# tooHotSpot/FGN

Measured on AMD Instinct MI355X. Metric: query-imgs/sec (3-way 3-shot, 800x1333 FGN simple_test), higher is better.
Workload: dtype f32; 1 GPU; cfg3: COCO2VOC 3-way 3-shot, query 3x800x1333, supports 9x3x256^2, ResNet-50-C4, R<=300 proposals, D<=100 detections, 1 episode(s) per GPU per step; h2d_in_step=True, gt_mask_rle_in_step=True, world_size_seen=1, phase_lock=rpn, caller_streams=2, support_cache=False, hip_graph=True, winograd_3x3=F(4x4,3x3)

## Files before the change

fgn_amd/csrc/common.h:

```cpp
#pragma once
#include <hip/hip_runtime.h>
#include <stdint.h>

#define FGN_OK 0
#define FGN_ERR_SHAPE (-1)
#define FGN_ERR_ARG (-2)

#define FGN_LAUNCH_CHECK()                         \
    do {                                           \
        hipError_t e__ = hipGetLastError();        \
        if (e__ != hipSuccess) return (int)e__;    \
    } while (0)

static inline int cdiv(int a, int b) { return (a + b - 1) / b; }

#include <hip/hip_ext.h>
extern thread_local hipEvent_t fgn_prof_start;
extern thread_local hipEvent_t fgn_prof_stop;
#define FGN_LAUNCH_TIMED(kernel, grid, block, lds, stream, ...)                                            \
    do {                                                                                                   \
        if (fgn_prof_start) {                                                                              \
            hipExtLaunchKernelGGL(kernel, grid, block, lds, stream, fgn_prof_start, fgn_prof_stop, 0, __VA_ARGS__); \
            fgn_prof_start = nullptr;                                                                      \
            fgn_prof_stop = nullptr;                                                                       \
        } else {                                                                                           \
            hipLaunchKernelGGL(kernel, grid, block, lds, stream, __VA_ARGS__);                             \
        }                                                                                                  \
    } while (0)

constexpr int FGN_STAMP_WORDS = 72;
extern thread_local unsigned long long* fgn_stamp_base;
extern thread_local int fgn_stamp_next, fgn_stamp_cap;
static inline unsigned long long* fgn_next_stamp_record() {
    if (!fgn_stamp_base || fgn_stamp_next >= fgn_stamp_cap) return nullptr;
    return fgn_stamp_base + FGN_STAMP_WORDS * (size_t)fgn_stamp_next++;
}

static inline hipError_t fgn_allow_full_lds(const void* fn, unsigned long long* done_mask) {
    int dev = 0;
    hipError_t e = hipGetDevice(&dev);
    if (e != hipSuccess) return e;
    if (dev < 64 && ((*done_mask >> dev) & 1ull)) return hipSuccess;
    e = hipFuncSetAttribute(fn, hipFuncAttributeMaxDynamicSharedMemorySize, 160 * 1024);
    if (e == hipSuccess && dev < 64) *done_mask |= 1ull << dev;
    return e;
}

typedef float f32x16 __attribute__((ext_vector_type(16)));
typedef float f32x4 __attribute__((ext_vector_type(4)));

__device__ __forceinline__ float wave_reduce_sum(float v) {
#pragma unroll
    for (int off = 32; off > 0; off >>= 1) v += __shfl_xor(v, off, 64);
    return v;
}
```

fgn_amd/csrc/conv_igemm.hip:

```cpp
#include "common.h"
#include <cstdlib>

struct ConvParams {
    const float* x = nullptr;
    const float* w = nullptr;
    float* y = nullptr;
    const float* scale = nullptr;
    const float* shift = nullptr;
    const float* residual = nullptr;
    const float* in_scale = nullptr;
    const int32_t* n_img_dev = nullptr;
    int n_img = 0, H = 1, W = 1, Cin = 0, Ho = 1, Wo = 1, Cout = 0, KH = 1, KW = 1, stride = 1, pad = 0;
    int a_img_div = 1;
    int relu = 0;
    int K = 0;
    int n_tiles_n = 0;
    int band_nt = 0, band_mt = 0;
    float* ws = nullptr;
    int splits = 1, kt_per_split = 0;
#ifdef FGN_EXPERIMENTS
    int32_t* tickets = nullptr;
    int32_t* sched = nullptr;
    int sk_U = 0, sk_dp = 0;
#endif
    unsigned x_bytes = 0, w_bytes = 0;
    int grp_rows = 0, grp_valid = 0, grp_items = 0, grp_rows_per_item = 0, grp_w_stride = 0;
    const int32_t* grp_count_dev = nullptr;
    unsigned long long* stamp = nullptr;
    const float* x2 = nullptr;
    unsigned x2_bytes = 0;
    int kt1 = 0, cin2 = 0;
    const int32_t* x2_rows = nullptr;
    const void* w3 = nullptr;
    unsigned w3_bytes = 0;
    int npad3 = 0;
    const float* w_inv = nullptr;
};

#ifndef CONV_DMA_STAGES
#define CONV_DMA_STAGES 2
#endif
constexpr int BK = 32;
constexpr int LDS_STRIDE = 36;

#ifdef CONV_CLOCK_STAMPS
__device__ unsigned long long g_clock_stamps[16384 * 6];
#define CLOCK_STAMP_BEGIN()                                                \
    const unsigned long long cs_t0 = __builtin_amdgcn_s_memtime();         \
    const unsigned long long cs_r0 = __builtin_amdgcn_s_memrealtime();     \
    __builtin_amdgcn_s_waitcnt(0xC07F)
#define CLOCK_STAMP_END(slot)                                              \
    do {                                                                   \
        const unsigned long long cs_t1 = __builtin_amdgcn_s_memtime();     \
        const unsigned long long cs_r1 = __builtin_amdgcn_s_memrealtime(); \
        __builtin_amdgcn_s_waitcnt(0xC07F);                                \
        unsigned cs_xcc, cs_hw;                                            \
        asm volatile("s_getreg_b32 %0, hwreg(HW_REG_XCC_ID)" : "=s"(cs_xcc)); \
        asm volatile("s_getreg_b32 %0, hwreg(HW_REG_HW_ID)" : "=s"(cs_hw));   \
        if (threadIdx.x == 0 && (slot) < 16384) {                          \
            g_clock_stamps[(slot) * 6 + 0] = cs_t0;                        \
            g_clock_stamps[(slot) * 6 + 1] = cs_t1;                        \
            g_clock_stamps[(slot) * 6 + 2] = cs_r0;                        \
            g_clock_stamps[(slot) * 6 + 3] = cs_r1;                        \
            g_clock_stamps[(slot) * 6 + 4] = cs_xcc;                       \
            g_clock_stamps[(slot) * 6 + 5] = cs_hw;                        \
        }                                                                  \
    } while (0)
#else
#define CLOCK_STAMP_BEGIN() do { } while (0)
#define CLOCK_STAMP_END(slot) do { } while (0)
#endif

template <int A_LD>
struct AStage {
    int off[A_LD];
    unsigned long long taps[A_LD];
    int soff[A_LD];
};

template <int N>
struct Pack {
    typedef float type __attribute__((ext_vector_type(N)));
};
#define PACK_SET4(pk, i, v)      \
    do {                         \
        (pk)[4 * (i) + 0] = (v).x; \
        (pk)[4 * (i) + 1] = (v).y; \
        (pk)[4 * (i) + 2] = (v).z; \
        (pk)[4 * (i) + 3] = (v).w; \
    } while (0)
#define PACK_GET4(pk, i) make_float4((pk)[4 * (i)], (pk)[4 * (i) + 1], (pk)[4 * (i) + 2], (pk)[4 * (i) + 3])

template <int A_LD, int B_LD, bool IN_SCALE>
__device__ __forceinline__ unsigned load_tile(const ConvParams& p, const AStage<A_LD>& st, const float* b_base,
                                              int kt, int cin_tiles, int col4,
                                              typename Pack<4 * A_LD>::type& a_reg,
                                              typename Pack<4 * A_LD>::type& s_reg,
                                              typename Pack<4 * B_LD>::type& b_reg) {
    unsigned ok_mask = 0;
    const int tap = kt / cin_tiles;
    const int c0 = (kt - tap * cin_tiles) * BK;
    const int ky = tap / p.KW, kx = tap - ky * p.KW;
    const int tap_off = (ky * p.W + kx) * p.Cin + c0;
#pragma unroll
    for (int i = 0; i < A_LD; ++i) {
        const bool ok = (st.taps[i] >> tap) & 1ull;
        const int off = ok ? st.off[i] + tap_off : 0;
        const float4 v = *reinterpret_cast<const float4*>(p.x + off);
        PACK_SET4(a_reg, i, v);
        if (IN_SCALE) {
            const float4 sv = *reinterpret_cast<const float4*>(p.in_scale + st.soff[i] + c0);
            PACK_SET4(s_reg, i, sv);
        }
        ok_mask |= ok ? (1u << i) : 0u;
    }
#pragma unroll
    for (int i = 0; i < B_LD; ++i) {
        const float4 v = *reinterpret_cast<const float4*>(b_base + (size_t)(32 * i) * p.K + kt * BK);
        PACK_SET4(b_reg, i, v);
    }
// ... 251 lines not shown
    constexpr unsigned OOB = 0x7ffffff0u;

    extern __shared__ __attribute__((aligned(16))) float smem[];

    const int t = threadIdx.x;
    const int lane = t & 63;
    const int wv = t >> 6;
    const int wm = wv / WAVES_N, wn = wv % WAVES_N;

    const int nwg = nwg_in;
    int bid = bx;
    {
        const int q = nwg >> 3, r = nwg & 7, xcd = bid & 7, idx = bid >> 3;
        bid = (xcd < r ? xcd * (q + 1) : r * (q + 1) + (xcd - r) * q) + idx;
    }
    int tile_m = bid / p.n_tiles_n;
    int tile_n = bid - tile_m * p.n_tiles_n;
    if (p.band_nt > 0) {
        const int per_grp = p.band_mt * p.n_tiles_n;
        const int grp = bid / per_grp;
        int r = bid - grp * per_grp;
        const int per_band = p.band_mt * p.band_nt;
        const int band = r / per_band;
        r -= band * per_band;
        const int mi = r / p.band_nt;
        tile_m = grp * p.band_mt + mi;
        tile_n = band * p.band_nt + (r - mi * p.band_nt);
    }
    const int m0 = tile_m * BM;
    const int n0 = tile_n * BN;

    const int HoWo = p.Ho * p.Wo;
    int n_img = p.n_img;
    if (p.n_img_dev) n_img = min(n_img, *p.n_img_dev);
    const int M = n_img * HoWo;
    if (m0 >= M) return;

    const int col4 = t & 7;
    const int row0 = t >> 3;
    const int src_c4 = col4 ^ ((row0 >> 1) & 7);
    int a_off[A_LD];
    unsigned long long a_taps[A_LD];
#pragma unroll
    for (int i = 0; i < A_LD; ++i) {
        const int m = m0 + row0 + 32 * i;
        a_off[i] = 0; a_taps[i] = 0ull;
        if (PW) {
            a_off[i] = (m * p.Cin + src_c4 * 4) * 4;
            a_taps[i] = m < M ? 1ull : 0ull;
        } else if (STEM) {
            if (m < M) {
                const int img = m / HoWo;
                const int rem = m - img * HoWo;
                const int oy = rem / p.Wo;
                const int ox = rem - oy * p.Wo;
                const int iy0 = oy * p.stride - p.pad, ix = ox * p.stride - p.pad + src_c4;
                a_off[i] = (((img / p.a_img_div) * p.H + iy0) * p.W + ix) * 16;
                unsigned long long tm = 0ull;
                if (src_c4 < p.KW && (unsigned)ix < (unsigned)p.W)
                    for (int ky = 0; ky < p.KH; ++ky)
                        if ((unsigned)(iy0 + ky) < (unsigned)p.H) tm |= 1ull << ky;
                a_taps[i] = tm;
            }
        } else if (m < M) {
            const int img = m / HoWo;
            const int rem = m - img * HoWo;
            const int oy = rem / p.Wo;
            const int ox = rem - oy * p.Wo;
            const int iy0 = oy * p.stride - p.pad, ix0 = ox * p.stride - p.pad;
            a_off[i] = ((((img / p.a_img_div) * p.H + iy0) * p.W + ix0) * p.Cin + src_c4 * 4) * 4;
            unsigned long long tm = 0ull;
            int tp = 0;
            for (int ky = 0; ky < p.KH; ++ky) {
                const bool y_ok = (unsigned)(iy0 + ky) < (unsigned)p.H;
                for (int kx = 0; kx < p.KW; ++kx, ++tp)
                    if (y_ok && (unsigned)(ix0 + kx) < (unsigned)p.W) tm |= 1ull << tp;
            }
            a_taps[i] = tm;
        }
    }
    int b_off0 = ((n0 + row0) * p.K + src_c4 * 4) * 4;
    if (PW && p.grp_rows) {
        const int grp = m0 / p.grp_rows;
        int valid = p.grp_valid;
        if (p.grp_count_dev) valid = min(valid, min(p.grp_items, *p.grp_count_dev) * p.grp_rows_per_item);
        if (m0 - grp * p.grp_rows >= valid) return;
        b_off0 += grp * p.grp_w_stride * 4;
    }

    const i32x4 x_rs = make_rsrc(p.x, p.x_bytes);
    const i32x4 w_rs = make_rsrc(p.w, p.w_bytes);

    const int KT_all = p.K / BK;
    const int kt0 = by * p.kt_per_split;
    const int KT = min(KT_all, kt0 + p.kt_per_split);
    const int cin_tiles = p.Cin / BK;

    const unsigned lds_base = __builtin_amdgcn_readfirstlane((unsigned)reinterpret_cast<size_t>(smem));
    const unsigned wave_row_bytes = __builtin_amdgcn_readfirstlane(wv) * 8 * 128;

    int nx_tap = 0, nx_c0t = 0, nx_kx = 0, nx_off = 0;
    if (!PW && !STEM) {
        nx_tap = kt0 / cin_tiles;
        nx_c0t = kt0 - nx_tap * cin_tiles;
        const int ky = nx_tap / p.KW;
        nx_kx = nx_tap - ky * p.KW;
        nx_off = ((ky * p.W + nx_kx) * p.Cin + nx_c0t * BK) * 4;
    }
    auto issue_tile = [&](int kt, int stage) {
        int tap = 0, tap_off = kt * BK * 4;
        if (STEM) {
            tap = kt;
            tap_off = kt * p.W * 16;
        } else if (!PW && NSTAGE == 2) {
            tap = nx_tap;
            tap_off = nx_off;
            nx_off += BK * 4;
            if (++nx_c0t == cin_tiles) {
                nx_c0t = 0;
                ++nx_tap;
                if (++nx_kx == p.KW) {
                    nx_kx = 0;
                    nx_off += (p.W - p.KW) * p.Cin * 4;
                }
            }
        } else if (!PW) {
            tap = kt / cin_tiles;
            const int c0 = (kt - tap * cin_tiles) * BK;
            const int ky = tap / p.KW, kx = tap - ky * p.KW;
            tap_off = ((ky * p.W + kx) * p.Cin + c0) * 4;
        }
        const unsigned sa = lds_base + stage * (STAGE * 4) + wave_row_bytes;
#pragma unroll
        for (int i = 0; i < A_LD; ++i) {
            const bool ok = (a_taps[i] >> tap) & 1ull;
            if (PW) {
                lds_dma16_s(x_rs, sa + i * 32 * 128, ok ? (unsigned)a_off[i] : OOB, (unsigned)tap_off);
                continue;
            }
            const unsigned voff = ok ? (unsigned)(a_off[i] + tap_off) : OOB;
            lds_dma16(x_rs, sa + i * 32 * 128, voff);
        }
        const unsigned sb = sa + BM * 128;
        const unsigned bko = (unsigned)(kt * BK * 4);
#pragma unroll
        for (int i = 0; i < B_LD; ++i)
            lds_dma16_s(w_rs, sb + i * 32 * 128, (unsigned)(b_off0 + i * 32 * p.K * 4), bko);
    };

    f32x16 acc[TM][TN];
#pragma unroll
    for (int i = 0; i < TM; ++i)
#pragma unroll
        for (int j = 0; j < TN; ++j)
#pragma unroll
            for (int r = 0; r < 16; ++r) acc[i][j][r] = 0.f;

    const int frag_row = lane & 31;
    const int half = lane >> 5;
    const int rswz = (frag_row >> 1) & 7;
    const float* const rd_a = smem + (wm * WM + frag_row) * BK;
    const float* const rd_b = smem + BM * BK + (wn * WN + frag_row) * BK;

#pragma unroll
    for (int s = 0; s < NSTAGE - 1; ++s) issue_tile(min(kt0 + s, KT - 1), s);
    if (NSTAGE == 2) asm volatile("s_waitcnt vmcnt(0)" ::: "memory");
    else asm volatile("s_waitcnt vmcnt(%0)" ::"n"(LOADS) : "memory");
    __builtin_amdgcn_s_barrier();
// ... 87 lines not shown
                        v.x = v.x * sc.x + sh.x; v.y = v.y * sc.y + sh.y; v.z = v.z * sc.z + sh.z; v.w = v.w * sc.w + sh.w;
                        v.x += res[k].x; v.y += res[k].y; v.z += res[k].z; v.w += res[k].w;
                        if (p.relu) {
                            v.x = fmaxf(v.x, 0.f); v.y = fmaxf(v.y, 0.f); v.z = fmaxf(v.z, 0.f); v.w = fmaxf(v.w, 0.f);
                        }
                    }
                    *reinterpret_cast<float4*>(dst + (size_t)m * p.Cout + n) = v;
                }
            }
        }
        return;
    }
    if (p.splits > 1) {
        float* slab = p.ws + (size_t)by * ((size_t)p.n_img * HoWo) * p.Cout;
#pragma unroll
        for (int j = 0; j < TN; ++j) {
            const int n = n0 + wn * WN + j * 32 + frag_row;
#pragma unroll
            for (int i = 0; i < TM; ++i) {
                const int mb = m0 + wm * WM + i * 32 + 4 * half;
#pragma unroll
                for (int r = 0; r < 16; ++r) {
                    const int m = mb + (r & 3) + 8 * (r >> 2);
                    if (n < p.Cout && m < M) slab[(size_t)m * p.Cout + n] = acc[i][j][r];
                }
            }
        }
        return;
    }
#pragma unroll
    for (int j = 0; j < TN; ++j) {
        const int n = n0 + wn * WN + j * 32 + frag_row;
        const bool n_ok = n < p.Cout;
        const float sc = (n_ok && p.scale) ? p.scale[n] : 1.f;
        const float sh = (n_ok && p.shift) ? p.shift[n] : 0.f;
#pragma unroll
        for (int i = 0; i < TM; ++i) {
            const int mb = m0 + wm * WM + i * 32 + 4 * half;
#pragma unroll
            for (int r = 0; r < 16; ++r) {
                const int m = mb + (r & 3) + 8 * (r >> 2);
                if (n_ok && m < M) {
                    const size_t o = (size_t)m * p.Cout + n;
                    float v = acc[i][j][r] * sc + sh;
                    if (p.residual) v += p.residual[o];
                    if (p.relu) v = fmaxf(v, 0.f);
                    p.y[o] = v;
                }
            }
        }
    }
}

template <int BM, int BN, int WM, int WN, int NSTAGE, int MIN_WAVES, int MODE>
__global__ __launch_bounds__(256, MIN_WAVES) void conv_igemm_dma_kernel(const ConvParams p) {
    CLOCK_STAMP_BEGIN();
    conv_igemm_dma_body<BM, BN, WM, WN, NSTAGE, MODE>(p, blockIdx.x, gridDim.x, blockIdx.y);
#ifdef CONV_CLOCK_STAMPS
    asm volatile("s_waitcnt vmcnt(0)" ::: "memory");
#endif
    CLOCK_STAMP_END(blockIdx.x);
}

template <int BM, int BN, int WM, int WN, int NSTAGE, int MIN_WAVES, int MODE>
__global__ __launch_bounds__(256, MIN_WAVES) void conv_igemm_dma_pair_kernel(const ConvParams p0, const ConvParams p1,
                                                                             const int n0) {
    if ((int)blockIdx.x < n0)
        conv_igemm_dma_body<BM, BN, WM, WN, NSTAGE, MODE>(p0, blockIdx.x, n0, 0);
    else
        conv_igemm_dma_body<BM, BN, WM, WN, NSTAGE, MODE>(p1, (int)blockIdx.x - n0, (int)gridDim.x - n0, 0);
}


__global__ __launch_bounds__(256, 5) void conv_pw_persist_kernel(const ConvParams p, const int total_tiles) {
    constexpr int BM = 64, BN = 64, WN = 32, WM = 32;
    constexpr int A_LD = 2, B_LD = 2;
    constexpr int STAGE = (BM + BN) * BK;
    constexpr int PITCH = BN;
    extern __shared__ __attribute__((aligned(16))) float smem[];

    const int t = threadIdx.x, lane = t & 63, wv = t >> 6;
    const int wm = wv >> 1, wn = wv & 1;
    const int M = (p.n_img_dev ? min(p.n_img, *p.n_img_dev) : p.n_img) * p.Ho * p.Wo;
    int grp_valid = p.grp_valid;
    if (p.grp_rows && p.grp_count_dev) grp_valid = min(grp_valid, min(p.grp_items, *p.grp_count_dev) * p.grp_rows_per_item);

    const int col4 = t & 7, row0 = t >> 3;
    const int src_c4 = col4 ^ ((row0 >> 1) & 7);
    const i32x4 x_rs = make_rsrc(p.x, p.x_bytes);
    const i32x4 w_rs = make_rsrc(p.w, p.w_bytes);
    const bool dual = p.x2 != nullptr;
    const i32x4 x2_rs = make_rsrc(dual ? p.x2 : p.x, dual ? p.x2_bytes : p.x_bytes);
    const int KT = p.K / BK;
    const unsigned lds_base = __builtin_amdgcn_readfirstlane((unsigned)reinterpret_cast<size_t>(smem));
    const unsigned wave_row_bytes = __builtin_amdgcn_readfirstlane(wv) * 8 * 128;
    constexpr unsigned OOB = 0x7ffffff0u;

    const int nq = total_tiles >> 3, nr = total_tiles & 7;
    auto coords = [&](int tile, int& m0, int& n0) -> bool {
        const int xcd = tile & 7, idx = tile >> 3;
        const int bid = (xcd < nr ? xcd * (nq + 1) : nr * (nq + 1) + (xcd - nr) * nq) + idx;
        int tile_m = bid / p.n_tiles_n;
        int tile_n = bid - tile_m * p.n_tiles_n;
        if (p.band_nt > 0) {
            const int per_grp = p.band_mt * p.n_tiles_n;
            const int grp = bid / per_grp;
            int r = bid - grp * per_grp;
            const int per_band = p.band_mt * p.band_nt;
            const int band = r / per_band;
            r -= band * per_band;
            const int mi = r / p.band_nt;
            tile_m = grp * p.band_mt + mi;
            tile_n = band * p.band_nt + (r - mi * p.band_nt);
        }
        m0 = tile_m * BM;
        n0 = tile_n * BN;
        if (m0 >= M) return false;
        if (p.grp_rows && m0 - (m0 / p.grp_rows) * p.grp_rows >= grp_valid) return false;
        return true;
    };
    auto next_active = [&](int tile, int& m0, int& n0) -> int {
        for (; tile < total_tiles; tile += gridDim.x)
            if (coords(tile, m0, n0)) return tile;
        return -1;
    };

    unsigned a_voff[A_LD], a2_voff[A_LD], b_voff[B_LD];
    auto set_offsets = [&](int m0, int n0) {
#pragma unroll
        for (int i = 0; i < A_LD; ++i) {
            const int m = m0 + row0 + 32 * i;
            a_voff[i] = m < M ? (unsigned)((m * p.Cin + src_c4 * 4) * 4) : OOB;
            a2_voff[i] = OOB;
            if (dual && m < M) a2_voff[i] = (unsigned)(((p.x2_rows ? p.x2_rows[m] : m) * p.cin2 + src_c4 * 4) * 4);
        }
        int b0 = ((n0 + row0) * p.K + src_c4 * 4) * 4;
        if (p.grp_rows) b0 += (m0 / p.grp_rows) * p.grp_w_stride * 4;
#pragma unroll
        for (int i = 0; i < B_LD; ++i) b_voff[i] = (unsigned)(b0 + i * 32 * p.K * 4);
    };
    auto issue_tile = [&](int kt, int stage) {
        const unsigned sa = lds_base + stage * (STAGE * 4) + wave_row_bytes;
        const unsigned ko = (unsigned)(kt * BK * 4);
        if (dual && kt >= p.kt1) {
            const unsigned ko2 = (unsigned)((kt - p.kt1) * BK * 4);
#pragma unroll
            for (int i = 0; i < A_LD; ++i) lds_dma16_s(x2_rs, sa + i * 32 * 128, a2_voff[i], ko2);
        } else {
#pragma unroll
            for (int i = 0; i < A_LD; ++i) lds_dma16_s(x_rs, sa + i * 32 * 128, a_voff[i], ko);
        }
        const unsigned sb = sa + BM * 128;
#pragma unroll
        for (int i = 0; i < B_LD; ++i) lds_dma16_s(w_rs, sb + i * 32 * 128, b_voff[i], ko);
    };

    const int r16 = lane & 15, g16 = lane >> 4;
    const float* const rd_a = smem + (wm * WM + r16) * BK;
    const float* const rd_b = smem + BM * BK + (wn * WN + r16) * BK;
    float* const cbase = smem + STAGE;

    if (p.stamp && t == 0 && blockIdx.x == 0) atomicExch(p.stamp, __builtin_amdgcn_s_memrealtime());
    auto leave = [&]() {
        if (!p.stamp || t != 0) return;
        const unsigned shard = blockIdx.x & 7u;
        const unsigned long long in_shard = (gridDim.x - shard + 7u) / 8u;
        unsigned long long* const sc = p.stamp + 8 * (1 + shard);
        if (atomicAdd(sc, 1ull) != in_shard - 1) return;
        atomicExch(sc, 0ull);
        const unsigned long long shards = gridDim.x < 8u ? gridDim.x : 8u;
        if (atomicAdd(p.stamp + 2, 1ull) != shards - 1) return;
        const unsigned long long d = __builtin_amdgcn_s_memrealtime() - atomicExch(p.stamp, 0ull);
        atomicExch(p.stamp + 2, 0ull);
        atomicAdd(p.stamp + 1, d);
        atomicAdd(p.stamp + 3, 1ull);
        atomicMin(p.stamp + 4, d);
        atomicMax(p.stamp + 5, d);
    };
    int m0, n0;
    int tile = next_active(blockIdx.x, m0, n0);
    if (tile < 0) { leave(); return; }
    CLOCK_STAMP_BEGIN();
    set_offsets(m0, n0);
    issue_tile(0, 0);

    while (true) {
        f32x4 acc4[2][2];
#pragma unroll
        for (int i = 0; i < 2; ++i)
#pragma unroll
            for (int j = 0; j < 2; ++j) acc4[i][j] = f32x4{0.f, 0.f, 0.f, 0.f};
        asm volatile("s_waitcnt vmcnt(0) lgkmcnt(0)" ::: "memory");
        __builtin_amdgcn_s_barrier();
        int cur = 0;
        for (int kt = 0; kt < KT; ++kt) {
            if (kt + 1 < KT) issue_tile(kt + 1, cur ^ 1);
            asm volatile("" ::: "memory");
            const float* As = rd_a + cur * STAGE;
            const float* Bs = rd_b + cur * STAGE;
#pragma unroll
            for (int kk = 0; kk < 2; ++kk) {
// ... 644 lines not shown
                                         const float* w_packed, float* y, const float* shift, int rows, int Cin1, int Cin2,
                                         int Cout, int cout_pad, int relu, hipStream_t stream) {
    ConvParams p;
    const int rc = describe_dual(p, MATH_F32, x, x2, x2_rows, x2_total_rows, w_packed, y, shift, rows, Cin1, Cin2, Cout, cout_pad, relu);
    if (rc != FGN_DESCRIBED) return rc;
    p.n_tiles_n = cdiv(Cout, 64);
    const int m_tiles = cdiv(rows, 64);
    set_band(p, 64, m_tiles, 64ll * p.K * 4);
    return launch_persist(p, m_tiles * p.n_tiles_n, stream);
}

extern "C" int fgn_conv1x1_dual_x3_nhwc_f32(const float* x, const float* x2, const int32_t* x2_rows, int x2_total_rows,
                                            const void* w_x3, float* y, const float* shift, int rows, int Cin1, int Cin2,
                                            int Cout, int cout_pad, int relu, hipStream_t stream) {
    ConvParams p;
    const int rc = describe_dual(p, MATH_X3, x, x2, x2_rows, x2_total_rows, w_x3, y, shift, rows, Cin1, Cin2, Cout, cout_pad, relu);
    if (rc != FGN_DESCRIBED) return rc;
    return launch_x3(p, rows, 0, 6, stream);
}

extern "C" int fgn_conv1x1_dual_h2_nhwc_f32(const float* x, const float* x2, const int32_t* x2_rows, int x2_total_rows,
                                            const void* w_h2, float* y, const float* shift, int rows, int Cin1, int Cin2,
                                            int Cout, int cout_pad, int relu, hipStream_t stream) {
    ConvParams p;
    const int rc = describe_dual(p, MATH_H2, x, x2, x2_rows, x2_total_rows, w_h2, y, shift, rows, Cin1, Cin2, Cout, cout_pad, relu);
    if (rc != FGN_DESCRIBED) return rc;
    return launch_h2(p, rows, 1, 0, stream);
}
extern "C" int fgn_conv1x1_dual_h2_bm_nhwc_f32(const float* x, const float* x2, const int32_t* x2_rows, int x2_total_rows,
                                               const void* w_h2, float* y, const float* shift, int rows, int Cin1, int Cin2,
                                               int Cout, int cout_pad, int relu, int bm, hipStream_t stream) {
    ConvParams p;
    const int rc = describe_dual(p, MATH_H2, x, x2, x2_rows, x2_total_rows, w_h2, y, shift, rows, Cin1, Cin2, Cout, cout_pad, relu);
    if (rc != FGN_DESCRIBED) return rc;
    return launch_h2(p, rows, 1, bm, stream);
}

static int describe_gemm(ConvParams& p, const GemmMath& m, const float* x, const void* w, float* y, const float* shift,
                         const float* residual, int rows, int K, int Cout, int npad, int relu, int grp_rows, int grp_valid,
                         int n_groups) {
    if (!x || !w || !y) return FGN_ERR_ARG;
    if (rows <= 0) return FGN_OK;
    if (K % BK || K <= 0 || (Cout & 3) || npad % m.bn || npad < Cout || n_groups < 1) return FGN_ERR_SHAPE;
    if (n_groups > 1 && (grp_rows <= 0 || (long long)n_groups * grp_rows != rows || grp_valid > grp_rows)) return FGN_ERR_SHAPE;
    const long long xb = (long long)rows * K * 4, wb = gemm_weight_bytes(m, K, npad, n_groups);
    if (xb >= 0x7fffff00ll || wb >= 0x7fffff00ll || (long long)rows * Cout >= (1ll << 31)) return FGN_ERR_SHAPE;
    p.x = x; p.y = y; p.shift = shift; p.residual = residual;
    p.n_img = rows; p.Cin = K; p.Cout = Cout; p.relu = relu; p.K = K; p.kt_per_split = K / BK; p.x_bytes = (unsigned)xb;
    p.grp_rows = n_groups > 1 ? grp_rows : 0; p.grp_valid = grp_valid;
    gemm_set_weights(p, m, w, wb, npad);
    return FGN_DESCRIBED;
}

extern "C" int fgn_gemm_x3_f32(const float* x, const void* w3, float* y, const float* shift, const float* residual,
                               int rows, int K, int Cout, int npad, int relu, int grp_rows, int grp_valid, int n_groups,
                               int bm, int nterms, hipStream_t stream) {
    ConvParams p;
    const int rc = describe_gemm(p, MATH_X3, x, w3, y, shift, residual, rows, K, Cout, npad, relu, grp_rows, grp_valid, n_groups);
    if (rc != FGN_DESCRIBED) return rc;
#ifdef X3_PHASES
    if (!g_x3_ph && (hipMalloc(&g_x3_ph, 256) != hipSuccess || hipMemset(g_x3_ph, 0, 256) != hipSuccess)) return FGN_ERR_ARG;
    p.ws = reinterpret_cast<float*>(g_x3_ph);
#endif
    return launch_x3(p, rows, bm, nterms, stream);
}

extern "C" int fgn_gemm_h2_f32(const float* x, const void* w_h2, float* y, const float* shift, const float* residual,
                               int rows, int K, int Cout, int npad, int relu, int grp_rows, int grp_valid, int n_groups,
                               int bm, hipStream_t stream) {
    ConvParams p;
    const int rc = describe_gemm(p, MATH_H2, x, w_h2, y, shift, residual, rows, K, Cout, npad, relu, grp_rows, grp_valid, n_groups);
    if (rc != FGN_DESCRIBED) return rc;
#ifdef H2_PHASES
    if (!g_x3_ph && (hipMalloc(&g_x3_ph, 256) != hipSuccess || hipMemset(g_x3_ph, 0, 256) != hipSuccess)) return FGN_ERR_ARG;
    p.ws = reinterpret_cast<float*>(g_x3_ph);
#endif
    return launch_h2(p, rows, n_groups, bm, stream);
}

extern "C" int fgn_winograd_t_pad(int tiles_total) { return (tiles_total + 127) / 128 * 128; }

static int describe_winograd_gemm(ConvParams& p, const GemmMath& m, const float* V, const void* U, float* Mo,
                                  const int32_t* n_img_dev, int n_img, int tiles_per_img, int t_pad, int Cin, int Cout,
                                  int cout_pad, int n_groups) {
    if (!V || !U || !Mo) return FGN_ERR_ARG;
    if (n_img <= 0) return FGN_OK;
    if (Cin % BK != 0 || (m.deep && Cin < 2 * BK) || Cout % 4 != 0 || cout_pad % m.bn != 0 || cout_pad < Cout || t_pad % 64 != 0 ||
        (n_groups != 16 && n_groups != 36) || (long long)n_img * tiles_per_img > t_pad)
        return FGN_ERR_SHAPE;
    const long long rows = (long long)n_groups * t_pad;
    const long long xb = rows * Cin * 4, wb = gemm_weight_bytes(m, Cin, cout_pad, n_groups);
    if (xb >= 0x7fffff00ll || wb >= 0x7fffff00ll || rows * Cout >= (1ll << 31)) return FGN_ERR_SHAPE;
    p.x = V; p.y = Mo;
    p.n_img = (int)rows; p.Cin = Cin; p.Cout = Cout; p.K = Cin; p.kt_per_split = Cin / BK; p.x_bytes = (unsigned)xb;
    p.grp_rows = t_pad; p.grp_valid = n_img * tiles_per_img; p.grp_items = n_img;
    p.grp_rows_per_item = tiles_per_img; p.grp_count_dev = n_img_dev;
    gemm_set_weights(p, m, U, wb, cout_pad);
    if (!m.image_bytes) p.grp_w_stride = cout_pad * Cin;
    return FGN_DESCRIBED;
}

extern "C" int fgn_winograd_gemm_f32(const float* V, const float* U, float* Mo, const int32_t* n_img_dev, int n_img,
                                     int tiles_per_img, int t_pad, int Cin, int Cout, int cout_pad, int n_groups,
                                     hipStream_t stream) {
    ConvParams p;
    const int rc = describe_winograd_gemm(p, MATH_F32, V, U, Mo, n_img_dev, n_img, tiles_per_img, t_pad, Cin, Cout, cout_pad, n_groups);
    if (rc != FGN_DESCRIBED) return rc;
#ifdef FGN_EXPERIMENTS
    {
        int rc2 = FGN_OK;
        if (fgn_exp_pointwise(p, p.n_img, 4, true, t_pad, stream, &rc2)) return rc2;
    }
#endif
    return launch_cfg<64, 64, 32, 32, 4>(p, p.n_img, pointwise_mode(4, p.n_img, Cout, 1), stream);
}

extern "C" int fgn_winograd_gemm_x3_f32(const float* V, const void* U_x3, float* Mo, const int32_t* n_img_dev, int n_img,
                                        int tiles_per_img, int t_pad, int Cin, int Cout, int cout_pad, int n_groups,
                                        hipStream_t stream) {
    ConvParams p;
    const int rc = describe_winograd_gemm(p, MATH_X3, V, U_x3, Mo, n_img_dev, n_img, tiles_per_img, t_pad, Cin, Cout, cout_pad, n_groups);
    if (rc != FGN_DESCRIBED) return rc;
    return launch_x3(p, p.n_img, 0, 6, stream);
}

extern "C" int fgn_winograd_gemm_h2_f32(const float* V, const void* U_h2, float* Mo, const int32_t* n_img_dev, int n_img,
                                        int tiles_per_img, int t_pad, int Cin, int Cout, int cout_pad, int n_groups,
                                        hipStream_t stream) {
    ConvParams p;
    const int rc = describe_winograd_gemm(p, MATH_H2, V, U_h2, Mo, n_img_dev, n_img, tiles_per_img, t_pad, Cin, Cout, cout_pad, n_groups);
    if (rc != FGN_DESCRIBED) return rc;
    return launch_h2(p, p.n_img, n_groups, 0, stream);
}
```

fgn_amd/csrc/conv_pw_h2.h:

```cpp
#pragma once

typedef _Float16 f16x8_t __attribute__((ext_vector_type(8)));

struct H2Frag { f16x8_t hi, lo; };

__device__ __forceinline__ void h2_split4(const float x0, const float x1, const float x2, const float x3, const float s,
                                          unsigned& h01, unsigned& h23, unsigned& l01, unsigned& l23) {
    asm("v_fma_mixlo_f16 %0, %4, %8, 0\n\t"
        "v_fma_mixlo_f16 %1, %6, %8, 0\n\t"
        "v_fma_mixhi_f16 %0, %5, %8, 0\n\t"
        "v_fma_mixhi_f16 %1, %7, %8, 0\n\t"
        "v_fma_mixlo_f16 %2, %4, %8, -%0 op_sel:[0,0,0] op_sel_hi:[0,0,1]\n\t"
        "v_fma_mixlo_f16 %3, %6, %8, -%1 op_sel:[0,0,0] op_sel_hi:[0,0,1]\n\t"
        "v_fma_mixhi_f16 %2, %5, %8, -%0 op_sel:[0,0,1] op_sel_hi:[0,0,1]\n\t"
        "v_fma_mixhi_f16 %3, %7, %8, -%1 op_sel:[0,0,1] op_sel_hi:[0,0,1]\n\t"
        "s_nop 1"
        : "=&v"(h01), "=&v"(h23), "=&v"(l01), "=&v"(l23)
        : "v"(x0), "v"(x1), "v"(x2), "v"(x3), "s"(s));
}

__device__ __forceinline__ void h2_split4_step(const int step, const float x0, const float x1, const float x2, const float x3,
                                               const float s, unsigned& h01, unsigned& h23, unsigned& l01, unsigned& l23) {
    if (step == 0)
        asm("v_fma_mixlo_f16 %0, %2, %4, 0\n\t"
// ... 13 lines not shown
            : "+v"(l01), "+v"(l23) : "v"(x1), "v"(x3), "s"(s), "v"(h01), "v"(h23));
}

__device__ __forceinline__ H2Frag h2_split(const float4& a, const float4& b, const float s) {
    unsigned h[4], l[4];
    h2_split4(a.x, a.y, a.z, a.w, s, h[0], h[1], l[0], l[1]);
    h2_split4(b.x, b.y, b.z, b.w, s, h[2], h[3], l[2], l[3]);
    H2Frag f;
    f.hi = __builtin_bit_cast(f16x8_t, make_uint4(h[0], h[1], h[2], h[3]));
    f.lo = __builtin_bit_cast(f16x8_t, make_uint4(l[0], l[1], l[2], l[3]));
    return f;
}

__device__ __forceinline__ float h2_absmax16(const float4& a, const float4& b, const float4& c, const float4& d) {
    float m;
    asm("v_max3_f32 %0, |%1|, |%2|, 0\n\t"
        "v_max3_f32 %0, |%3|, |%4|, %0\n\t"
        "v_max3_f32 %0, |%5|, |%6|, %0\n\t"
        "v_max3_f32 %0, |%7|, |%8|, %0\n\t"
        "v_max3_f32 %0, |%9|, |%10|, %0\n\t"
        "v_max3_f32 %0, |%11|, |%12|, %0\n\t"
        "v_max3_f32 %0, |%13|, |%14|, %0\n\t"
        "v_max3_f32 %0, |%15|, |%16|, %0"
        : "=&v"(m)
        : "v"(a.x), "v"(a.y), "v"(a.z), "v"(a.w), "v"(b.x), "v"(b.y), "v"(b.z), "v"(b.w),
          "v"(c.x), "v"(c.y), "v"(c.z), "v"(c.w), "v"(d.x), "v"(d.y), "v"(d.z), "v"(d.w));
    return m;
}

constexpr int H2_BN = 128;

struct H2Im2col {
    float* y1;
    unsigned x_off0, x_off1;
    int M0, M1;
    int H1, W1, Ho1, Wo1;
    int cin_shift;
};

#ifdef H2_PHASES
#define H2_T(i) do { const unsigned long long now_ = __builtin_amdgcn_s_memtime(); ph_[i] += now_ - last_; last_ = now_; } while (0)
#else
#define H2_T(i) do { } while (0)
#endif
struct H2Yes { static constexpr bool value = true; };
struct H2No { static constexpr bool value = false; };
constexpr int H2_ONE = 0, H2_TWO = 1, H2_EITHER = 2;
template <int WMW, int WNW, int RB, int NST, bool IM2COL, int KG, int DUAL>
__device__ __forceinline__ void conv_pw_h2_body(const ConvParams p, const H2Im2col q2, const int total_tiles) {
    static_assert(!(DUAL != H2_ONE && IM2COL), "the implicit-GEMM loader reads one operand");
    constexpr int BM = 32 * RB * WMW, BN = 64 * WNW, NW = WMW * WNW, NTHR_G = 64 * NW, NTHR = NTHR_G * KG;
    static_assert(KG == 1 || KG == 2, "one or two K-groups");
    constexpr int A_LD = BM / 8 / NW;
    constexpr int A_STAGE = BM * 128;
    constexpr int B_STAGE = 2 * BN * 64;
    constexpr int STAGE = A_STAGE + B_STAGE;
    constexpr int BQ = BN / 16;
    constexpr int B_LD = 2 * BQ / NW;
    static_assert(A_LD * 8 * NW == BM && B_LD * NW == 2 * BQ, "tile / wave split");
    constexpr int PER = A_LD + B_LD;
    constexpr int ROWS_PER_PASS = NTHR_G / 8;
    constexpr bool OLD_CURSOR = KG == 2 && !IM2COL;
#ifdef H2_EPILOGUE_PASSES
    constexpr bool WPE = false;
#else
    constexpr bool WPE = KG == 1;
#endif
#ifdef H2_PHASES
    constexpr bool PEEL = true;
#else
    constexpr bool PEEL = WPE;
#endif
    constexpr int C_LD = 68;
    static_assert(!WPE || NW * 16 * C_LD * 4 <= STAGE, "a 16-row block per wave fits the free stage");
    static_assert(NST == 2, "a ring of two stages: one K-tile in flight ahead of the one being multiplied");
    extern __shared__ __attribute__((aligned(16))) unsigned char smem_h2[];

    const int t = threadIdx.x, lane = t & 63;
    const int kg = KG == 1 ? 0 : __builtin_amdgcn_readfirstlane((t >> 6) / NW);
    const int wv = KG == 1 ? t >> 6 : (t >> 6) % NW;
    const int tg = KG == 1 ? t : t % NTHR_G;
    const int wm = wv / WNW, wn = wv % WNW;
    const int M = IM2COL ? q2.M0 + q2.M1 : (p.n_img_dev ? min(p.n_img, *p.n_img_dev) : p.n_img) * p.Ho * p.Wo;
    int grp_valid = p.grp_valid;
    if (p.grp_rows && p.grp_count_dev) grp_valid = min(grp_valid, min(p.grp_items, *p.grp_count_dev) * p.grp_rows_per_item);

    float a_s = 1.f, a_inv = 1.f;

    const int col4 = tg & 7, row0 = tg >> 3;
    const int src_c4 = col4 ^ ((row0 >> 1) & 7);
    const i32x4 x_rs = make_rsrc(p.x, p.x_bytes);
    const i32x4 w_rs = make_rsrc(p.w3, p.w3_bytes);
    [[maybe_unused]] const bool dual = DUAL == H2_EITHER ? p.x2 != nullptr : DUAL == H2_TWO;
    [[maybe_unused]] const i32x4 x2_rs = DUAL != H2_ONE ? make_rsrc(dual ? p.x2 : p.x, dual ? p.x2_bytes : p.x_bytes) : x_rs;
    const int KT = p.K / BK / KG;
    const unsigned kt_bytes = (unsigned)(2 * p.npad3 * 64);
    const unsigned lds_base = __builtin_amdgcn_readfirstlane((unsigned)reinterpret_cast<size_t>(smem_h2) + kg * (NST * STAGE));
    const unsigned wave_row_bytes = __builtin_amdgcn_readfirstlane(wv) * 8 * 128;
    constexpr unsigned OOB = 0x7ffffff0u;

    const int nq = total_tiles >> 3, nr = total_tiles & 7;
    auto coords = [&](int tile, int& m0, int& n0) -> bool {
        const int xcd = tile & 7, idx = tile >> 3;
        const int bid = (xcd < nr ? xcd * (nq + 1) : nr * (nq + 1) + (xcd - nr) * nq) + idx;
        int tile_m = bid / p.n_tiles_n;
        int tile_n = bid - tile_m * p.n_tiles_n;
        if (p.band_nt > 0) {
            const int per_grp = p.band_mt * p.n_tiles_n;
            const int grp = bid / per_grp;
            int r = bid - grp * per_grp;
            const int per_band = p.band_mt * p.band_nt;
            const int band = r / per_band;
            r -= band * per_band;
            const int mi = r / p.band_nt;
            tile_m = grp * p.band_mt + mi;
            tile_n = band * p.band_nt + (r - mi * p.band_nt);
        }
        m0 = tile_m * BM;
        n0 = tile_n * BN;
        if (m0 >= M) return false;
        if (p.grp_rows && m0 - (m0 / p.grp_rows) * p.grp_rows >= grp_valid) return false;
        return true;
    };
    auto next_active = [&](int tile, int& m0, int& n0) -> int {
        for (; tile < total_tiles; tile += gridDim.x)
            if (coords(tile, m0, n0)) return tile;
        return -1;
    };

    constexpr int A2_LD = (IM2COL || DUAL != H2_ONE) ? A_LD : 1;
    struct Offs { unsigned a[A_LD], a2[A2_LD], b[B_LD]; };
    unsigned b_lds[B_LD];
#pragma unroll
    for (int i = 0; i < B_LD; ++i) {
        const int q = wv + NW * i;
        b_lds[i] = __builtin_amdgcn_readfirstlane((unsigned)(A_STAGE + (q / BQ) * (BN * 64) + (q % BQ) * 1024));
    }
    auto offsets = [&](int m0, int n0) -> Offs {
        Offs o;
        o.a2[0] = 0u;
        const int g_end = p.grp_rows ? (m0 / p.grp_rows) * p.grp_rows + grp_valid : M;
#pragma unroll
        for (int i = 0; i < A_LD; ++i) {
            const int m = m0 + row0 + ROWS_PER_PASS * i;
            if constexpr (IM2COL) {
                o.a[i] = 0u; o.a2[i] = 0u;
                if (m < M) {
                    const bool t1 = m >= q2.M0;
                    const int mm = t1 ? m - q2.M0 : m;
                    const int H = t1 ? q2.H1 : p.H, W = t1 ? q2.W1 : p.W, Wo = t1 ? q2.Wo1 : p.Wo;
                    const int HoWo = (t1 ? q2.Ho1 : p.Ho) * Wo;
                    const int img = mm / HoWo;
                    const int rem = mm - img * HoWo;
                    const int oy = rem / Wo;
                    const int ox = rem - oy * Wo;
                    const int iy0 = oy * p.stride - p.pad, ix0 = ox * p.stride - p.pad;
                    o.a[i] = (t1 ? q2.x_off1 : q2.x_off0) + (unsigned)((((img * H + iy0) * W + ix0) * p.Cin + src_c4 * 4) * 4);
                    unsigned tm = t1 ? 0x80000000u : 0u;
                    int tp = 0;
                    for (int ky = 0; ky < p.KH; ++ky) {
                        const bool y_ok = (unsigned)(iy0 + ky) < (unsigned)H;
                        for (int kx = 0; kx < p.KW; ++kx, ++tp)
                            if (y_ok && (unsigned)(ix0 + kx) < (unsigned)W) tm |= 1u << tp;
                    }
                    o.a2[i] = tm;
                }
                continue;
            }
            const bool in = m < M && m < g_end;
            o.a[i] = in ? (unsigned)((m * p.Cin + src_c4 * 4) * 4) : OOB;
            if constexpr (DUAL != H2_ONE) {
                o.a2[i] = OOB;
                if (dual && in) o.a2[i] = (unsigned)(((p.x2_rows ? p.x2_rows[m] : m) * p.cin2 + src_c4 * 4) * 4);
            }
        }
        unsigned g0 = 0;
        if (p.grp_rows) g0 = (unsigned)(m0 / p.grp_rows) * (unsigned)(KT * KG) * kt_bytes;
#pragma unroll
        for (int i = 0; i < B_LD; ++i) {
            const int q = wv + NW * i;
            const int plane = q / BQ, row = (q % BQ) * 16 + (lane >> 2);
            o.b[i] = g0 + (unsigned)(((plane * p.npad3 + n0 + row) * 4 + (lane & 3)) * 16);
        }
        return o;
    };
    const unsigned ko_step = (unsigned)(KG * BK * 4), kb_step = (unsigned)KG * kt_bytes;
    [[maybe_unused]] const unsigned ko1 = (DUAL != H2_ONE && dual) ? (unsigned)(p.kt1 * BK * 4) : 0xffffffffu;
    unsigned c_ko = 0u, c_kb = 0u;
    int c_tap = 0, c_cs = 0, c_kx = 0;
    unsigned c_off0 = 0u, c_off1 = 0u;
    const int im_ct = 1 << q2.cin_shift;
    const unsigned im_skip0 = (unsigned)((p.W - p.KW) * p.Cin * 4), im_skip1 = (unsigned)((q2.W1 - p.KW) * p.Cin * 4);
    auto seek = [&](int step) {
        const int kt = step * KG + kg;
        c_ko = (unsigned)(kt * BK * 4);
        c_kb = (unsigned)kt * kt_bytes;
        if constexpr (IM2COL) {
            c_tap = kt >> q2.cin_shift;
            c_cs = kt - (c_tap << q2.cin_shift);
            const int ky = p.KW == 3 ? (c_tap * 43) >> 7 : c_tap;
            c_kx = c_tap - ky * p.KW;
            c_off0 = (unsigned)(((ky * p.W + c_kx) * p.Cin + c_cs * BK) * 4);
            c_off1 = (unsigned)(((ky * q2.W1 + c_kx) * p.Cin + c_cs * BK) * 4);
        }
    };
    auto advance = [&]() {
        c_ko += ko_step;
        c_kb += kb_step;
        if constexpr (IM2COL) {
#pragma unroll
            for (int g = 0; g < KG; ++g) {
                const bool tw = ++c_cs == im_ct;
                c_cs = tw ? 0 : c_cs;
                c_tap += tw;
                c_kx += tw;
                const bool rw = c_kx == p.KW;
                c_kx = rw ? 0 : c_kx;
                c_off0 += 128u + (rw ? im_skip0 : 0u);
                c_off1 += 128u + (rw ? im_skip1 : 0u);
            }
        }
    };
    auto piece = [&](const Offs& o, const unsigned wr, const int idx) {
        const unsigned st = lds_base + wr;
// ... 419 lines not shown
```

fgn_amd/csrc/conv_pw_x3.h:

```cpp
#pragma once

typedef __bf16 bf16x8_t __attribute__((ext_vector_type(8)));

struct X3Frag { bf16x8_t p1, p2, p3; };

__device__ __forceinline__ X3Frag x3_split(const float4& lo, const float4& hi) {
    const float x[8] = {lo.x, lo.y, lo.z, lo.w, hi.x, hi.y, hi.z, hi.w};
    unsigned q1[4], q2[4], q3[4];
#pragma unroll
    for (int i = 0; i < 4; ++i) {
        const unsigned u0 = __float_as_uint(x[2 * i]), u1 = __float_as_uint(x[2 * i + 1]);
        q1[i] = __builtin_amdgcn_perm(u1, u0, 0x07060302u);
        const float r0 = x[2 * i] - __uint_as_float(u0 & 0xffff0000u);
        const float r1 = x[2 * i + 1] - __uint_as_float(u1 & 0xffff0000u);
        const unsigned v0 = __float_as_uint(r0), v1 = __float_as_uint(r1);
        q2[i] = __builtin_amdgcn_perm(v1, v0, 0x07060302u);
        const float s0 = r0 - __uint_as_float(v0 & 0xffff0000u);
        const float s1 = r1 - __uint_as_float(v1 & 0xffff0000u);
        q3[i] = __builtin_amdgcn_perm(__float_as_uint(s1), __float_as_uint(s0), 0x07060302u);
    }
    X3Frag f;
    f.p1 = __builtin_bit_cast(bf16x8_t, make_uint4(q1[0], q1[1], q1[2], q1[3]));
    f.p2 = __builtin_bit_cast(bf16x8_t, make_uint4(q2[0], q2[1], q2[2], q2[3]));
    f.p3 = __builtin_bit_cast(bf16x8_t, make_uint4(q3[0], q3[1], q3[2], q3[3]));
    return f;
}

constexpr int X3_BN = 128;
constexpr int X3_B_STAGE = 3 * X3_BN * 64;

#ifdef X3_PHASES
#define X3_T(i) do { const unsigned long long now_ = __builtin_amdgcn_s_memtime(); ph_[i] += now_ - last_; last_ = now_; } while (0)
#else
#define X3_T(i) do { } while (0)
#endif

template <int N> __device__ __forceinline__ void x3_wait_vm() { asm volatile("s_waitcnt vmcnt(%0)" ::"n"(N) : "memory"); }

template <int WMW, int RB, int NT, int NST, bool SH16>
__global__ __launch_bounds__(128 * WMW, 2) void conv_pw_x3_kernel(const ConvParams p, const int total_tiles) {
    constexpr int BM = 32 * RB * WMW, BN = X3_BN, NTHR = 128 * WMW, NW = 2 * WMW;
    constexpr int A_LD = BM / 8 / NW;
    constexpr int A_STAGE = BM * 128;
    constexpr int STAGE = A_STAGE + X3_B_STAGE;
    constexpr int B_LD = 24 / NW;
    constexpr int PER = A_LD + B_LD;
    constexpr int D = NST - 1;
    constexpr int ROWS_PER_PASS = NTHR / 8;
    static_assert(NST == 2 || NST == 3, "ring of 2 or 3 stages");
    extern __shared__ __attribute__((aligned(16))) unsigned char smem_x3[];

    const int t = threadIdx.x, lane = t & 63, wv = t >> 6;
    const int wm = wv >> 1, wn = wv & 1;
    const int M = (p.n_img_dev ? min(p.n_img, *p.n_img_dev) : p.n_img) * p.Ho * p.Wo;
    int grp_valid = p.grp_valid;
    if (p.grp_rows && p.grp_count_dev) grp_valid = min(grp_valid, min(p.grp_items, *p.grp_count_dev) * p.grp_rows_per_item);

    const int col4 = t & 7, row0 = t >> 3;
    const int src_c4 = col4 ^ ((row0 >> 1) & 7);
    const i32x4 x_rs = make_rsrc(p.x, p.x_bytes);
    const i32x4 w_rs = make_rsrc(p.w3, p.w3_bytes);
    const bool dual = p.x2 != nullptr;
    const i32x4 x2_rs = make_rsrc(dual ? p.x2 : p.x, dual ? p.x2_bytes : p.x_bytes);
    const int KT = p.K / BK;
    const unsigned kt_bytes = (unsigned)(3 * p.npad3 * 64);
    const unsigned lds_base = __builtin_amdgcn_readfirstlane((unsigned)reinterpret_cast<size_t>(smem_x3));
    const unsigned wave_row_bytes = __builtin_amdgcn_readfirstlane(wv) * 8 * 128;
    constexpr unsigned OOB = 0x7ffffff0u;

    const int nq = total_tiles >> 3, nr = total_tiles & 7;
    auto coords = [&](int tile, int& m0, int& n0) -> bool {
        const int xcd = tile & 7, idx = tile >> 3;
        const int bid = (xcd < nr ? xcd * (nq + 1) : nr * (nq + 1) + (xcd - nr) * nq) + idx;
        int tile_m = bid / p.n_tiles_n;
        int tile_n = bid - tile_m * p.n_tiles_n;
        if (p.band_nt > 0) {
            const int per_grp = p.band_mt * p.n_tiles_n;
            const int grp = bid / per_grp;
            int r = bid - grp * per_grp;
            const int per_band = p.band_mt * p.band_nt;
            const int band = r / per_band;
            r -= band * per_band;
            const int mi = r / p.band_nt;
            tile_m = grp * p.band_mt + mi;
            tile_n = band * p.band_nt + (r - mi * p.band_nt);
        }
        m0 = tile_m * BM;
        n0 = tile_n * BN;
        if (m0 >= M) return false;
        if (p.grp_rows && m0 - (m0 / p.grp_rows) * p.grp_rows >= grp_valid) return false;
        return true;
    };
    auto next_active = [&](int tile, int& m0, int& n0) -> int {
        for (; tile < total_tiles; tile += gridDim.x)
            if (coords(tile, m0, n0)) return tile;
        return -1;
    };

    struct Offs { unsigned a[A_LD], a2[A_LD], b[B_LD]; };
    unsigned b_lds[B_LD];
#pragma unroll
    for (int i = 0; i < B_LD; ++i) {
        const int q = wv + NW * i;
        b_lds[i] = __builtin_amdgcn_readfirstlane((unsigned)(A_STAGE + (q >> 3) * (BN * 64) + (q & 7) * 1024));
    }
    auto offsets = [&](int m0, int n0) -> Offs {
        Offs o;
#pragma unroll
        for (int i = 0; i < A_LD; ++i) {
            const int m = m0 + row0 + ROWS_PER_PASS * i;
            o.a[i] = m < M ? (unsigned)((m * p.Cin + src_c4 * 4) * 4) : OOB;
            o.a2[i] = OOB;
            if (dual && m < M) o.a2[i] = (unsigned)(((p.x2_rows ? p.x2_rows[m] : m) * p.cin2 + src_c4 * 4) * 4);
        }
        unsigned g0 = 0;
        if (p.grp_rows) g0 = (unsigned)(m0 / p.grp_rows) * (unsigned)KT * kt_bytes;
#pragma unroll
        for (int i = 0; i < B_LD; ++i) {
            const int q = wv + NW * i;
            const int plane = q >> 3, row = (q & 7) * 16 + (lane >> 2);
            o.b[i] = g0 + (unsigned)(((plane * p.npad3 + n0 + row) * 4 + (lane & 3)) * 16);
        }
        return o;
    };
    auto issue = [&](const Offs& o, int kt, int stage) {
        const unsigned st = lds_base + stage * STAGE;
        const unsigned sa = st + wave_row_bytes;
        const unsigned ko = (unsigned)(kt * BK * 4);
        if (dual && kt >= p.kt1) {
            const unsigned ko2 = (unsigned)((kt - p.kt1) * BK * 4);
#pragma unroll
            for (int i = 0; i < A_LD; ++i) lds_dma16_s(x2_rs, sa + i * ROWS_PER_PASS * 128, o.a2[i], ko2);
        } else {
#pragma unroll
            for (int i = 0; i < A_LD; ++i) lds_dma16_s(x_rs, sa + i * ROWS_PER_PASS * 128, o.a[i], ko);
        }
        const unsigned kb = (unsigned)kt * kt_bytes;
#pragma unroll
        for (int i = 0; i < B_LD; ++i) lds_dma16_s(w_rs, st + b_lds[i], o.b[i], kb);
    };

    const int r32 = lane & 31, h = lane >> 5;
    const int a_row = wm * 32 * RB + r32;
    const unsigned a_sw = (unsigned)((a_row >> 1) & 7);
    unsigned a_rd[2][2], b_rd[2][2];
#pragma unroll
    for (int s = 0; s < 2; ++s) {
        const unsigned ca = (unsigned)(4 * s + 2 * h);
        a_rd[s][0] = (unsigned)(a_row * 128) + ((ca ^ a_sw) << 4);
        a_rd[s][1] = (unsigned)(a_row * 128) + (((ca + 1) ^ a_sw) << 4);
#pragma unroll
        for (int j = 0; j < 2; ++j) {
            const int n = wn * 64 + 32 * j + r32;
            b_rd[s][j] = (unsigned)(A_STAGE + n * 64) + ((((unsigned)(2 * s + h)) ^ (unsigned)((n >> 2) & 3)) << 4);
        }
    }

    const int r16 = lane & 15, g4 = lane >> 4;
    const int a16_row = wm * 32 * RB + r16;
    const unsigned a16_sw = (unsigned)((a16_row >> 1) & 7);
    const unsigned a16_rd0 = (unsigned)(a16_row * 128) + ((((unsigned)g4) ^ a16_sw) << 4);
    const unsigned a16_rd1 = (unsigned)(a16_row * 128) + ((((unsigned)(g4 + 4)) ^ a16_sw) << 4);
    const int n16 = wn * 64 + r16;
    const unsigned tau16 = (0x1230u >> (4 * ((n16 >> 2) & 3))) & 3u;
    const unsigned b16_rd = (unsigned)(A_STAGE + n16 * 64) + ((((unsigned)g4) ^ tau16) << 4);

    if (p.stamp && t == 0 && blockIdx.x == 0) atomicExch(p.stamp, __builtin_amdgcn_s_memrealtime());
    auto leave = [&]() {
        if (!p.stamp || t != 0) return;
        const unsigned shard = blockIdx.x & 7u;
        const unsigned long long in_shard = (gridDim.x - shard + 7u) / 8u;
        unsigned long long* const sc = p.stamp + 8 * (1 + shard);
        if (atomicAdd(sc, 1ull) != in_shard - 1) return;
// ... 233 lines not shown
```

fgn_amd/csrc/winograd.hip:

```cpp
#include "common.h"
#include <cstdlib>

__device__ __forceinline__ float4 f4add(float4 a, float4 b) { return make_float4(a.x + b.x, a.y + b.y, a.z + b.z, a.w + b.w); }
__device__ __forceinline__ float4 f4sub(float4 a, float4 b) { return make_float4(a.x - b.x, a.y - b.y, a.z - b.z, a.w - b.w); }
__device__ __forceinline__ float4 f4mul(float4 a, float4 b) { return make_float4(a.x * b.x, a.y * b.y, a.z * b.z, a.w * b.w); }

__global__ __launch_bounds__(256) void wg_input_kernel(const float4* __restrict__ x, const float4* __restrict__ in_scale,
                                                       float4* __restrict__ V, const int32_t* __restrict__ n_img_dev,
                                                       int n_img, int a_img_div, int H, int W, int C4, int ty, int tx,
                                                       int t_pad, long long total) {
    if (n_img_dev) n_img = min(n_img, *n_img_dev);
    for (long long i = blockIdx.x * (long long)blockDim.x + threadIdx.x; i < total;
         i += (long long)gridDim.x * blockDim.x) {
        const int c = (int)(i % C4);
        const int t = (int)(i / C4);
        const int xx = t % tx;
        const int r = t / tx;
        const int yy = r % ty;
        const int img = r / ty;
        if (img >= n_img) break;
        const float4* src = x + (size_t)(img / a_img_div) * H * W * C4 + c;
        const int iy0 = 2 * yy - 1, ix0 = 2 * xx - 1;
        float4 d[4][4];
#pragma unroll
// ... 85 lines not shown
    if (n_img <= 0) return FGN_OK;
    const int ty = (H + 1) / 2, tx = (W + 1) / 2;
    if (C % 4 != 0 || a_img_div < 1 || H < 1 || W < 1 || (long long)n_img * ty * tx > t_pad) return FGN_ERR_SHAPE;
    const long long total = (long long)n_img * ty * tx * (C / 4);
    const int grid = (int)std::min<long long>((total + 255) / 256, 256 * 32);
    FGN_LAUNCH_TIMED(wg_input_kernel, dim3(grid), dim3(256), 0, stream, reinterpret_cast<const float4*>(x),
                       reinterpret_cast<const float4*>(in_scale), reinterpret_cast<float4*>(V), n_img_dev, n_img,
                       a_img_div, H, W, C / 4, ty, tx, t_pad, total);
    FGN_LAUNCH_CHECK();
    return FGN_OK;
}

extern "C" int fgn_winograd_output_f32(const float* Mo, float* y, const float* shift, const int32_t* n_img_dev,
                                       int n_img, int H, int W, int C, int t_pad, int relu, hipStream_t stream) {
    if (!Mo || !y) return FGN_ERR_ARG;
    if (n_img <= 0) return FGN_OK;
    const int ty = (H + 1) / 2, tx = (W + 1) / 2;
    if (C % 4 != 0 || (long long)n_img * ty * tx > t_pad) return FGN_ERR_SHAPE;
    const long long total = (long long)n_img * ty * tx * (C / 4);
    const int grid = (int)std::min<long long>((total + 255) / 256, 256 * 32);
    FGN_LAUNCH_TIMED(wg_output_kernel, dim3(grid), dim3(256), 0, stream, reinterpret_cast<const float4*>(Mo),
                       reinterpret_cast<float4*>(y), reinterpret_cast<const float4*>(shift), n_img_dev, n_img, H, W,
                       C / 4, ty, tx, t_pad, relu, total);
    FGN_LAUNCH_CHECK();
    return FGN_OK;
}

template <int V>
struct VF {
    typedef float type __attribute__((ext_vector_type(V)));
};
template <int V>
using vf = typename VF<V>::type;

template <int V>
__device__ __forceinline__ vf<V> vfma(float k, vf<V> a, vf<V> acc) {
    vf<V> r;
#pragma unroll
    for (int i = 0; i < V; ++i) r[i] = fmaf(k, a[i], acc[i]);
    return r;
}
template <int V>
__device__ __forceinline__ vf<V> vmul_rn(vf<V> a, vf<V> s) {
#pragma clang fp contract(off)
    return a * s;
}
template <int V>
__device__ __forceinline__ vf<V> vzero() {
    vf<V> r;
#pragma unroll
    for (int i = 0; i < V; ++i) r[i] = 0.f;
    return r;
}
template <int V>
__device__ __forceinline__ vf<V> vrelu(vf<V> a) {
#pragma unroll
    for (int i = 0; i < V; ++i) a[i] = fmaxf(a[i], 0.f);
    return a;
}
template <int V>
__device__ __forceinline__ void wg4_bt(const vf<V> (&d)[6], vf<V> (&r)[6]) {
    r[0] = (vfma<V>(1.5f, d[3] - d[1], vfma<V>(-2.f, d[2], d[0]))) + d[4];
    r[1] = vfma<V>(2.5f, d[3], vfma<V>(0.5f, d[2], d[4] - d[1]));
    r[2] = vfma<V>(0.5f, d[3], vfma<V>(-2.5f, d[2], d[1] + d[4]));
    r[3] = vfma<V>(2.f, d[3] - d[1], d[4] - d[2]);
    r[4] = vfma<V>(0.5f, d[1] - d[3], d[4] - d[2]);
    r[5] = (vfma<V>(1.5f, d[4] - d[2], vfma<V>(-2.f, d[3], d[1]))) + d[5];
}
template <int V>
__device__ __forceinline__ void wg4_at(const vf<V> (&m)[6], vf<V> (&r)[4]) {
    const vf<V> s12 = m[1] + m[2], d12 = m[1] - m[2];
    r[0] = (m[0] + s12) + (m[3] + m[4]);
    r[1] = vfma<V>(-2.f, m[4], vfma<V>(0.5f, m[3], d12));
    r[2] = vfma<V>(4.f, m[4], vfma<V>(0.25f, m[3], s12));
    r[3] = (vfma<V>(-8.f, m[4], vfma<V>(0.125f, m[3], d12))) + m[5];
}

struct WgSeg {
    const float* x;
    int n_img, H, W, ty, tx;
    int tiles0;
};

template <int V, bool EAGER>
__global__ __launch_bounds__(256) void wg4_input_kernel(const float* __restrict__ x_, const float* __restrict__ in_scale_,
                                                        float* __restrict__ V_, const int32_t* __restrict__ n_img_dev,
                                                        int n_img, int a_img_div, int H, int W, int CV, int ty, int tx,
                                                        int t_pad, long long total, const WgSeg seg) {
    typedef vf<V> T;
    const T* __restrict__ x = reinterpret_cast<const T*>(x_);
    const T* __restrict__ in_scale = reinterpret_cast<const T*>(in_scale_);
    T* __restrict__ Vo = reinterpret_cast<T*>(V_);
    if (n_img_dev) n_img = min(n_img, *n_img_dev);
    for (long long i = blockIdx.x * (long long)blockDim.x + threadIdx.x; i < total;
         i += (long long)gridDim.x * blockDim.x) {
        const int c = (int)(i % CV);
        const int t = (int)(i / CV);
        const bool second = seg.x && t >= seg.tiles0;
        if (second) {
            x = reinterpret_cast<const T*>(seg.x);
            H = seg.H; W = seg.W; ty = seg.ty; tx = seg.tx; n_img = seg.n_img; a_img_div = 1;
        }
        const int tl = second ? t - seg.tiles0 : t;
        const int xx = tl % tx;
        const int r = tl / tx;
        const int yy = r % ty;
        const int img = r / ty;
        if (img >= n_img) {
            if (seg.x) continue;
            break;
        }
        const T* src = x + (size_t)(img / a_img_div) * H * W * CV + c;
        const int iy0 = 4 * yy - 1, ix0 = 4 * xx - 1;
        T s;
        if (in_scale) s = in_scale[(size_t)img * CV + c];
        else {
#pragma unroll
            for (int k = 0; k < V; ++k) s[k] = 1.f;
        }
        T tt[6][6];
        if (EAGER) {
#pragma unroll
            for (int a = 0; a < 6; ++a) {
                const int iy = iy0 + a;
#pragma unroll
                for (int b = 0; b < 6; ++b) {
                    const int ix = ix0 + b;
                    tt[a][b] = ((unsigned)iy < (unsigned)H && (unsigned)ix < (unsigned)W)
                                   ? src[((size_t)iy * W + ix) * CV] : vzero<V>();
                }
            }
#pragma unroll
            for (int b = 0; b < 6; ++b) {
                T d[6], rr[6];
#pragma unroll
                for (int a = 0; a < 6; ++a) d[a] = vmul_rn<V>(tt[a][b], s);
                wg4_bt<V>(d, rr);
#pragma unroll
                for (int a = 0; a < 6; ++a) tt[a][b] = rr[a];
            }
        } else {
#pragma unroll
            for (int b = 0; b < 6; ++b) {
                const int ix = ix0 + b;
                T d[6], rr[6];
#pragma unroll
                for (int a = 0; a < 6; ++a) {
                    const int iy = iy0 + a;
                    d[a] = ((unsigned)iy < (unsigned)H && (unsigned)ix < (unsigned)W)
                               ? vmul_rn<V>(src[((size_t)iy * W + ix) * CV], s) : vzero<V>();
                }
                wg4_bt<V>(d, rr);
#pragma unroll
                for (int a = 0; a < 6; ++a) tt[a][b] = rr[a];
            }
        }
        T* dst = Vo + (size_t)t * CV + c;
        const size_t gs = (size_t)t_pad * CV;
#pragma unroll
        for (int a = 0; a < 6; ++a) {
            T rr[6];
            wg4_bt<V>(tt[a], rr);
#pragma unroll
            for (int b = 0; b < 6; ++b) dst[(a * 6 + b) * gs] = rr[b];
        }
    }
}

template <int V>
__global__ __launch_bounds__(256) void wg4_output_kernel(const float* __restrict__ Mo_, float* __restrict__ y_,
                                                         const float* __restrict__ shift_,
                                                         const int32_t* __restrict__ n_img_dev, int n_img, int H, int W,
                                                         int CV, int ty, int tx, int t_pad, int relu, long long total,
                                                         const WgSeg seg) {
    typedef vf<V> T;
    const T* __restrict__ Mo = reinterpret_cast<const T*>(Mo_);
    const T* __restrict__ shift = reinterpret_cast<const T*>(shift_);
    T* __restrict__ y = reinterpret_cast<T*>(y_);
    if (n_img_dev) n_img = min(n_img, *n_img_dev);
    for (long long i = blockIdx.x * (long long)blockDim.x + threadIdx.x; i < total;
         i += (long long)gridDim.x * blockDim.x) {
        const int c = (int)(i % CV);
        const int t = (int)(i / CV);
        const bool second = seg.x && t >= seg.tiles0;
        if (second) {
            y = reinterpret_cast<T*>(const_cast<float*>(seg.x));
            H = seg.H; W = seg.W; ty = seg.ty; tx = seg.tx; n_img = seg.n_img;
        }
        const int tl = second ? t - seg.tiles0 : t;
        const int xx = tl % tx;
        const int r = tl / tx;
        const int yy = r % ty;
        const int img = r / ty;
        if (img >= n_img) {
            if (seg.x) continue;
            break;
        }
        const T* src = Mo + (size_t)t * CV + c;
        const size_t gs = (size_t)t_pad * CV;
        T mm[6][6];
#pragma unroll
        for (int a = 0; a < 6; ++a)
#pragma unroll
            for (int b = 0; b < 6; ++b) mm[a][b] = src[(a * 6 + b) * gs];
        T st[4][6];
#pragma unroll
        for (int b = 0; b < 6; ++b) {
            T m[6], rr[4];
#pragma unroll
            for (int a = 0; a < 6; ++a) m[a] = mm[a][b];
            wg4_at<V>(m, rr);
#pragma unroll
            for (int k = 0; k < 4; ++k) st[k][b] = rr[k];
        }
        const T sh = shift ? shift[c] : vzero<V>();
#pragma unroll
        for (int a = 0; a < 4; ++a) {
            const int oy = 4 * yy + a;
            T rr[4];
            wg4_at<V>(st[a], rr);
            if (oy >= H) continue;
#pragma unroll
            for (int b = 0; b < 4; ++b) {
                const int ox = 4 * xx + b;
                if (ox >= W) continue;
                T v = rr[b] + sh;
                if (relu) v = vrelu<V>(v);
                y[(((size_t)img * H + oy) * W + ox) * CV + c] = v;
            }
        }
    }
}

struct WgDiv {
    uint32_t mul, shift;
};
static WgDiv wg_div(uint32_t d) {
    WgDiv r = {0u, 0u};
    if (d > 1) {
        const int L = 32 - __builtin_clz(d - 1);
        r.mul = (uint32_t)(((1ull << (31 + L)) + d - 1) / d);
        r.shift = (uint32_t)(L - 1);
    }
    return r;
}
__device__ __forceinline__ uint32_t wg_quot(uint32_t n, WgDiv d) { return d.mul ? __umulhi(n, d.mul) >> d.shift : n; }

struct WgMap {
    const float* p;
    int H, W;
    int n_img;
    uint32_t ty, tx;
    WgDiv dty, dtx;
    uint32_t elems;
};
struct WgNarrow {
    WgMap m[2];
    uint32_t blocks0;
    uint32_t tiles0;
    uint32_t CV;
    WgDiv dcv, ddiv;
    uint32_t gs;
};

template <typename T>
__device__ __forceinline__ T wg_ld(const void* base, uint32_t off) {
    return *reinterpret_cast<const T*>(static_cast<const char*>(base) + off);
}
template <typename T>
__device__ __forceinline__ void wg_st(void* base, uint32_t off, T v) {
    *reinterpret_cast<T*>(static_cast<char*>(base) + off) = v;
}

__device__ __forceinline__ int wg_count_early(const int32_t* n_img_dev) {
    if (!n_img_dev) return 0x7fffffff;
    const int32_t* p = n_img_dev;
    asm volatile("" : "+v"(p));
    return *p;
}

template <int V>
__global__ __launch_bounds__(256) void wg4_input_narrow_kernel(const WgNarrow P, const float* __restrict__ in_scale,
                                                               float* __restrict__ Vo, const int32_t* __restrict__ n_img_dev) {
    typedef vf<V> T;
    const int dev_count = wg_count_early(n_img_dev);
    const bool second = blockIdx.x >= P.blocks0;
    const float* __restrict__ x = second ? P.m[1].p : P.m[0].p;
    const int H = second ? P.m[1].H : P.m[0].H, W = second ? P.m[1].W : P.m[0].W;
    const uint32_t ty = second ? P.m[1].ty : P.m[0].ty, tx = second ? P.m[1].tx : P.m[0].tx;
    const WgDiv dty = second ? P.m[1].dty : P.m[0].dty, dtx = second ? P.m[1].dtx : P.m[0].dtx;
    const uint32_t elems = second ? P.m[1].elems : P.m[0].elems;
    const int n_cap = second ? P.m[1].n_img : P.m[0].n_img;
    const uint32_t i = (blockIdx.x - (second ? P.blocks0 : 0u)) * 256u + threadIdx.x;
    if (i >= elems) return;
    const uint32_t tl = wg_quot(i, P.dcv), c = i - tl * P.CV;
    const uint32_t r = wg_quot(tl, dtx), xx = tl - r * tx;
    const uint32_t img = wg_quot(r, dty), yy = r - img * ty;
    const uint32_t t = tl + (second ? P.tiles0 : 0u);
    const uint32_t px = (uint32_t)sizeof(T) * P.CV;
    const int iy0 = 4 * (int)yy - 1, ix0 = 4 * (int)xx - 1;
    uint32_t ro[6], co[6];
    bool rok[6], cok[6];
    const uint32_t row0 = wg_quot(img, P.ddiv) * (uint32_t)H;
#pragma unroll
    for (int a = 0; a < 6; ++a) {
        const int iy = iy0 + a, ix = ix0 + a;
        rok[a] = (unsigned)iy < (unsigned)H;
        cok[a] = (unsigned)ix < (unsigned)W;
        ro[a] = (row0 + (uint32_t)min(max(iy, 0), H - 1)) * (uint32_t)W * px;
        co[a] = (uint32_t)min(max(ix, 0), W - 1) * px + c * (uint32_t)sizeof(T);
    }
    T tt[6][6];
#pragma unroll
    for (int a = 0; a < 6; ++a)
#pragma unroll
        for (int b = 0; b < 6; ++b) tt[a][b] = wg_ld<T>(x, ro[a] + co[b]);
    T s;
    if (in_scale) s = wg_ld<T>(in_scale, (img * P.CV + c) * (uint32_t)sizeof(T));
    else {
#pragma unroll
        for (int k = 0; k < V; ++k) s[k] = 1.f;
    }
#pragma unroll
    for (int b = 0; b < 6; ++b) {
        T d[6], rr[6];
#pragma unroll
        for (int a = 0; a < 6; ++a) d[a] = vmul_rn<V>((rok[a] && cok[b]) ? tt[a][b] : vzero<V>(), s);
        wg4_bt<V>(d, rr);
#pragma unroll
        for (int a = 0; a < 6; ++a) tt[a][b] = rr[a];
    }
    if ((int)img >= min(n_cap, dev_count)) return;
    uint32_t o = (t * P.CV + c) * (uint32_t)sizeof(T);
#pragma unroll
    for (int a = 0; a < 6; ++a) {
        T rr[6];
        wg4_bt<V>(tt[a], rr);
#pragma unroll
        for (int b = 0; b < 6; ++b) {
            wg_st<T>(Vo, o, rr[b]);
            o += P.gs;
        }
    }
}

template <int V>
__global__ __launch_bounds__(256) void wg4_output_narrow_kernel(const WgNarrow P, const float* __restrict__ Mo,
                                                                const float* __restrict__ shift,
                                                                const int32_t* __restrict__ n_img_dev, int relu) {
    typedef vf<V> T;
    const int dev_count = wg_count_early(n_img_dev);
    const bool second = blockIdx.x >= P.blocks0;
    float* __restrict__ y = const_cast<float*>(second ? P.m[1].p : P.m[0].p);
    const int H = second ? P.m[1].H : P.m[0].H, W = second ? P.m[1].W : P.m[0].W;
    const uint32_t ty = second ? P.m[1].ty : P.m[0].ty, tx = second ? P.m[1].tx : P.m[0].tx;
    const WgDiv dty = second ? P.m[1].dty : P.m[0].dty, dtx = second ? P.m[1].dtx : P.m[0].dtx;
    const uint32_t elems = second ? P.m[1].elems : P.m[0].elems;
    const int n_cap = second ? P.m[1].n_img : P.m[0].n_img;
    const uint32_t i = (blockIdx.x - (second ? P.blocks0 : 0u)) * 256u + threadIdx.x;
    if (i >= elems) return;
    const uint32_t tl = wg_quot(i, P.dcv), c = i - tl * P.CV;
    const uint32_t t = tl + (second ? P.tiles0 : 0u);
    T mm[6][6];
    {
        uint32_t o = (t * P.CV + c) * (uint32_t)sizeof(T);
#pragma unroll
        for (int a = 0; a < 6; ++a)
#pragma unroll
            for (int b = 0; b < 6; ++b) {
                mm[a][b] = wg_ld<T>(Mo, o);
                o += P.gs;
            }
    }
    const T sh = shift ? wg_ld<T>(shift, c * (uint32_t)sizeof(T)) : vzero<V>();
    const uint32_t r = wg_quot(tl, dtx), xx = tl - r * tx;
    const uint32_t img = wg_quot(r, dty), yy = r - img * ty;
    T st[4][6];
#pragma unroll
    for (int b = 0; b < 6; ++b) {
        T m[6], rr[4];
#pragma unroll
        for (int a = 0; a < 6; ++a) m[a] = mm[a][b];
        wg4_at<V>(m, rr);
#pragma unroll
        for (int k = 0; k < 4; ++k) st[k][b] = rr[k];
    }
    if ((int)img >= min(n_cap, dev_count)) return;
    const uint32_t px = (uint32_t)sizeof(T) * P.CV;
    const uint32_t oy0 = 4u * yy, ox0 = 4u * xx;
    uint32_t orow = ((img * (uint32_t)H + oy0) * (uint32_t)W + ox0) * px + c * (uint32_t)sizeof(T);
#pragma unroll
    for (int a = 0; a < 4; ++a) {
        T rr[4];
        wg4_at<V>(st[a], rr);
        if ((int)(oy0 + a) < H) {
#pragma unroll
            for (int b = 0; b < 4; ++b) {
                if ((int)(ox0 + b) >= W) continue;
                T v = rr[b] + sh;
                if (relu) v = vrelu<V>(v);
                wg_st<T>(y, orow + b * px, v);
            }
        }
        orow += (uint32_t)W * px;
    }
}

static int wg4_vec(long long elems) { return elems >= (4ll << 20) ? 4 : 2; }
static bool wg4_eager(long long) { return true; }
extern "C" int fgn_winograd4_variant(int tiles_total, int C, int is_output) {
    const int v = wg4_vec((long long)tiles_total * C);
    return v * 10 + ((!is_output && wg4_eager((long long)tiles_total * (C / v))) ? 1 : 0);
}

static bool wg4_narrow_fits(long long imgs0, int H0, int W0, long long imgs1, int H1, int W1, long long n_scale, int C,
                            int t_pad) {
    const long long lim = 0x7fffffffll, cb = 4ll * C;
    return imgs0 * H0 * W0 * cb <= lim && imgs1 * H1 * W1 * cb <= lim && n_scale * cb <= lim && 36ll * t_pad * cb <= lim;
}
static void wg4_map(WgMap& m, const float* p, int n_img, int H, int W, int cv) {
    m.p = p; m.H = H; m.W = W; m.n_img = n_img;
    m.ty = (uint32_t)(H + 3) / 4; m.tx = (uint32_t)(W + 3) / 4;
    m.dty = wg_div(m.ty); m.dtx = wg_div(m.tx);
    m.elems = p ? (uint32_t)n_img * m.ty * m.tx * (uint32_t)cv : 0u;
}
static WgNarrow wg4_narrow(const float* p0, int n_img0, int a_img_div, int H0, int W0, const float* p1, int n_img1, int H1,
                           int W1, int C, int vec, int t_pad, int* grid) {
    WgNarrow P;
    const int cv = C / vec;
    wg4_map(P.m[0], p0, n_img0, H0, W0, cv);
    wg4_map(P.m[1], p1, n_img1, H1, W1, cv);
    P.blocks0 = (P.m[0].elems + 255u) / 256u;
    P.tiles0 = (uint32_t)n_img0 * P.m[0].ty * P.m[0].tx;
    P.CV = (uint32_t)cv;
    P.dcv = wg_div(P.CV);
    P.ddiv = wg_div((uint32_t)a_img_div);
    P.gs = (uint32_t)t_pad * (uint32_t)C * 4u;
    *grid = (int)(P.blocks0 + (P.m[1].elems + 255u) / 256u);
    return P;
}
static bool wg4_takes_narrow(bool is_output, int n_img, int a_img_div, int H, int W, int n_img1, int H1, int W1, int C,
                             int t_pad, bool with_scale, int vec_force) {
    if (a_img_div < 1 || C < 4) return false;
    const long long tiles_all = (long long)n_img * ((H + 3) / 4) * ((W + 3) / 4) + (long long)n_img1 * ((H1 + 3) / 4) * ((W1 + 3) / 4);
    const int vec = vec_force ? vec_force : wg4_vec(tiles_all * C);
    if (!is_output && !wg4_eager(tiles_all * (C / vec))) return false;
    const long long imgs0 = is_output ? n_img : (n_img + a_img_div - 1) / a_img_div;
    return wg4_narrow_fits(imgs0, H, W, n_img1, H1, W1, (!is_output && with_scale) ? n_img : 0, C, t_pad);
}
extern "C" int fgn_winograd4_index_bits(int n_img, int a_img_div, int H, int W, int n_img1, int H1, int W1, int C, int t_pad,
                                        int with_scale, int is_output) {
    return wg4_takes_narrow(is_output != 0, n_img, a_img_div, H, W, n_img1, H1, W1, C, t_pad, with_scale != 0, 0) ? 32 : 64;
}

#define WG4_IN_LAUNCH(VV, EE)                                                                                          \
    FGN_LAUNCH_TIMED((wg4_input_kernel<VV, EE>), dim3(grid), dim3(256), 0, stream, x, in_scale, V, n_img_dev, n_img,  \
                     a_img_div, H, W, C / VV, ty, tx, t_pad, total, seg)
#define WG4_IN_NARROW(VV)                                                                                              \
    FGN_LAUNCH_TIMED((wg4_input_narrow_kernel<VV>), dim3(ngrid), dim3(256), 0, stream, P, in_scale, V, n_img_dev)

static int wg4_input_launch(const float* x, const float* in_scale, float* V, const int32_t* n_img_dev, int n_img,
                            int a_img_div, int H, int W, int C, int t_pad, const float* x1, int n_img1, int H1, int W1,
                            int index_bits, int vec_force, hipStream_t stream) {
    if (!x || !V) return FGN_ERR_ARG;
    if (index_bits != 0 && index_bits != 32 && index_bits != 64) return FGN_ERR_ARG;
    if (vec_force != 0 && vec_force != 1 && vec_force != 2 && vec_force != 4) return FGN_ERR_ARG;
    if (n_img <= 0) return FGN_OK;
    const int ty = (H + 3) / 4, tx = (W + 3) / 4;
    WgSeg seg;
    seg.x = x1; seg.n_img = n_img1; seg.H = H1; seg.W = W1; seg.ty = (H1 + 3) / 4; seg.tx = (W1 + 3) / 4;
    seg.tiles0 = n_img * ty * tx;
    const long long tiles_all = (long long)seg.tiles0 + (x1 ? (long long)n_img1 * seg.ty * seg.tx : 0);
    if (C % 4 != 0 || a_img_div < 1 || H < 1 || W < 1 || tiles_all > t_pad) return FGN_ERR_SHAPE;
    if (x1 && (in_scale || n_img_dev || a_img_div != 1 || n_img1 < 1 || H1 < 1 || W1 < 1)) return FGN_ERR_SHAPE;
    const int vec = vec_force ? vec_force : wg4_vec(tiles_all * C);
    const long long total = tiles_all * (C / vec);
    const bool eager = wg4_eager(total);
    const bool fits = wg4_takes_narrow(false, n_img, a_img_div, H, W, x1 ? n_img1 : 0, H1, W1, C, t_pad, in_scale != nullptr, vec_force);
    if (index_bits == 32 && !fits) return FGN_ERR_SHAPE;
    if (fits && index_bits != 64) {
        int ngrid = 0;
        const WgNarrow P = wg4_narrow(x, n_img, a_img_div, H, W, x1, n_img1, H1, W1, C, vec, t_pad, &ngrid);
        switch (vec) {
            case 1: WG4_IN_NARROW(1); break;
            case 2: WG4_IN_NARROW(2); break;
            default: WG4_IN_NARROW(4); break;
        }
        FGN_LAUNCH_CHECK();
        return FGN_OK;
    }
    const int grid = (int)std::min<long long>((total + 255) / 256, 256 * 32);
    switch (vec * 10 + (eager ? 1 : 0)) {
        case 11: WG4_IN_LAUNCH(1, true); break;
        case 10: WG4_IN_LAUNCH(1, false); break;
        case 21: WG4_IN_LAUNCH(2, true); break;
        case 20: WG4_IN_LAUNCH(2, false); break;
        case 41: WG4_IN_LAUNCH(4, true); break;
        default: WG4_IN_LAUNCH(4, false); break;
    }
    FGN_LAUNCH_CHECK();
    return FGN_OK;
}

extern "C" int fgn_winograd4_input_f32(const float* x, const float* in_scale, float* V, const int32_t* n_img_dev,
                                       int n_img, int a_img_div, int H, int W, int C, int t_pad, hipStream_t stream) {
    return wg4_input_launch(x, in_scale, V, n_img_dev, n_img, a_img_div, H, W, C, t_pad, nullptr, 0, 1, 1, 0, 0, stream);
}
extern "C" int fgn_winograd4_input2_f32(const float* x0, int n_img0, int H0, int W0, const float* x1, int n_img1, int H1,
                                        int W1, float* V, int C, int t_pad, hipStream_t stream) {
    if (!x1) return FGN_ERR_ARG;
    return wg4_input_launch(x0, nullptr, V, nullptr, n_img0, 1, H0, W0, C, t_pad, x1, n_img1, H1, W1, 0, 0, stream);
}
extern "C" int fgn_winograd4_input_ix_f32(const float* x, const float* in_scale, float* V, const int32_t* n_img_dev,
                                          int n_img, int a_img_div, int H, int W, int C, int t_pad, const float* x1,
                                          int n_img1, int H1, int W1, int index_bits, int vec, hipStream_t stream) {
    return wg4_input_launch(x, in_scale, V, n_img_dev, n_img, a_img_div, H, W, C, t_pad, x1, x1 ? n_img1 : 0, x1 ? H1 : 1,
                            x1 ? W1 : 1, index_bits, vec, stream);
}

#define WG4_OUT_LAUNCH(VV)                                                                                             \
    FGN_LAUNCH_TIMED((wg4_output_kernel<VV>), dim3(grid), dim3(256), 0, stream, Mo, y, shift, n_img_dev, n_img, H, W, \
                     C / VV, ty, tx, t_pad, relu, total, seg)
#define WG4_OUT_NARROW(VV)                                                                                             \
    FGN_LAUNCH_TIMED((wg4_output_narrow_kernel<VV>), dim3(ngrid), dim3(256), 0, stream, P, Mo, shift, n_img_dev, relu)

static int wg4_output_launch(const float* Mo, float* y, const float* shift, const int32_t* n_img_dev, int n_img, int H,
                             int W, int C, int t_pad, int relu, float* y1, int n_img1, int H1, int W1, int index_bits,
                             int vec_force, hipStream_t stream) {
    if (!Mo || !y) return FGN_ERR_ARG;
    if (index_bits != 0 && index_bits != 32 && index_bits != 64) return FGN_ERR_ARG;
    if (vec_force != 0 && vec_force != 1 && vec_force != 2 && vec_force != 4) return FGN_ERR_ARG;
    if (n_img <= 0) return FGN_OK;
    const int ty = (H + 3) / 4, tx = (W + 3) / 4;
    WgSeg seg;
    seg.x = y1; seg.n_img = n_img1; seg.H = H1; seg.W = W1; seg.ty = (H1 + 3) / 4; seg.tx = (W1 + 3) / 4;
    seg.tiles0 = n_img * ty * tx;
    const long long tiles_all = (long long)seg.tiles0 + (y1 ? (long long)n_img1 * seg.ty * seg.tx : 0);
    if (C % 4 != 0 || H < 1 || W < 1 || tiles_all > t_pad) return FGN_ERR_SHAPE;
    if (y1 && (n_img_dev || n_img1 < 1 || H1 < 1 || W1 < 1)) return FGN_ERR_SHAPE;
    const int vec = vec_force ? vec_force : wg4_vec(tiles_all * C);
    const long long total = tiles_all * (C / vec);
    const bool fits = wg4_takes_narrow(true, n_img, 1, H, W, y1 ? n_img1 : 0, H1, W1, C, t_pad, false, vec_force);
    if (index_bits == 32 && !fits) return FGN_ERR_SHAPE;
    if (fits && index_bits != 64) {
        int ngrid = 0;
        const WgNarrow P = wg4_narrow(y, n_img, 1, H, W, y1, n_img1, H1, W1, C, vec, t_pad, &ngrid);
        switch (vec) {
            case 1: WG4_OUT_NARROW(1); break;
            case 2: WG4_OUT_NARROW(2); break;
            default: WG4_OUT_NARROW(4); break;
        }
        FGN_LAUNCH_CHECK();
        return FGN_OK;
    }
    const int grid = (int)std::min<long long>((total + 255) / 256, 256 * 32);
    switch (vec) {
        case 1: WG4_OUT_LAUNCH(1); break;
        case 2: WG4_OUT_LAUNCH(2); break;
        default: WG4_OUT_LAUNCH(4); break;
    }
    FGN_LAUNCH_CHECK();
    return FGN_OK;
}

extern "C" int fgn_winograd4_output_f32(const float* Mo, float* y, const float* shift, const int32_t* n_img_dev,
                                        int n_img, int H, int W, int C, int t_pad, int relu, hipStream_t stream) {
    return wg4_output_launch(Mo, y, shift, n_img_dev, n_img, H, W, C, t_pad, relu, nullptr, 0, 1, 1, 0, 0, stream);
}
extern "C" int fgn_winograd4_output2_f32(const float* Mo, const float* shift, float* y0, int n_img0, int H0, int W0,
                                         float* y1, int n_img1, int H1, int W1, int C, int t_pad, int relu,
                                         hipStream_t stream) {
    if (!y1) return FGN_ERR_ARG;
    return wg4_output_launch(Mo, y0, shift, nullptr, n_img0, H0, W0, C, t_pad, relu, y1, n_img1, H1, W1, 0, 0, stream);
}
extern "C" int fgn_winograd4_output_ix_f32(const float* Mo, float* y, const float* shift, const int32_t* n_img_dev,
                                           int n_img, int H, int W, int C, int t_pad, int relu, float* y1, int n_img1,
                                           int H1, int W1, int index_bits, int vec, hipStream_t stream) {
    return wg4_output_launch(Mo, y, shift, n_img_dev, n_img, H, W, C, t_pad, relu, y1, y1 ? n_img1 : 0, y1 ? H1 : 1,
                             y1 ? W1 : 1, index_bits, vec, stream);
}

template <int R>
__global__ __launch_bounds__(256) void wg_pack_weights_kernel(const float* __restrict__ w, const double* __restrict__ G,
                                                              float* __restrict__ U, int cout, int cin, int cout_pad) {
    __shared__ double g[R][3];
    if (threadIdx.x < R * 3) g[threadIdx.x / 3][threadIdx.x % 3] = G[threadIdx.x];
    __syncthreads();
    const long long total = (long long)cout * cin;
    for (long long q = blockIdx.x * (long long)blockDim.x + threadIdx.x; q < total; q += (long long)gridDim.x * blockDim.x) {
        const int co = (int)(q / cin), ci = (int)(q - (long long)co * cin);
        double k[3][3];
#pragma unroll
        for (int i = 0; i < 9; ++i) k[i / 3][i % 3] = (double)w[q * 9 + i];
        double t[R][3];
#pragma unroll
        for (int a = 0; a < R; ++a)
#pragma unroll
            for (int j = 0; j < 3; ++j) t[a][j] = g[a][0] * k[0][j] + g[a][1] * k[1][j] + g[a][2] * k[2][j];
#pragma unroll
        for (int a = 0; a < R; ++a)
#pragma unroll
            for (int b = 0; b < R; ++b)
                U[((size_t)(a * R + b) * cout_pad + co) * cin + ci] =
                    (float)(t[a][0] * g[b][0] + t[a][1] * g[b][1] + t[a][2] * g[b][2]);
    }
}

extern "C" int fgn_winograd_pack_weights_f32(const float* w, const double* G, float* U, int cout, int cin, int cout_pad,
                                             int m, hipStream_t stream) {
    if (!w || !G || !U) return FGN_ERR_ARG;
    if ((m != 2 && m != 4) || cout < 1 || cin < 1 || cout_pad < cout) return FGN_ERR_SHAPE;
    const long long total = (long long)cout * cin;
    const int grid = (int)std::min<long long>((total + 255) / 256, 256 * 16);
    if (m == 4)
        hipLaunchKernelGGL(wg_pack_weights_kernel<6>, dim3(grid), dim3(256), 0, stream, w, G, U, cout, cin, cout_pad);
    else
        hipLaunchKernelGGL(wg_pack_weights_kernel<4>, dim3(grid), dim3(256), 0, stream, w, G, U, cout, cin, cout_pad);
    FGN_LAUNCH_CHECK();
    return FGN_OK;
}
```

fgn_amd/lib.py:

```python
from __future__ import annotations

import ctypes as C
import os

_HERE = os.path.dirname(os.path.abspath(__file__))
LIB_PATH = os.environ.get('FGN_HIP_LIB') or os.path.join(_HERE, 'libfgn_hip.so')

_p = C.c_void_p
_i = C.c_int
_f = C.c_float

SIGNATURES = {
    'fgn_abi_version': (_i, []),
    'fgn_profile_next_launch': (_i, [_p, _p]),
    'fgn_profile_stamp_words': (_i, []),
    'fgn_profile_stamps': (_i, [_p, _i]),
    'fgn_phase_signal': (_i, [_p, _p]),
    'fgn_phase_wait': (_i, [_p, _i, _i, _p]),
    'fgn_conv2d_workspace_bytes': (C.c_size_t, [_i] * 10),
    'fgn_conv2d_kernel_id': (_i, [_i] * 14),
    'fgn_conv2d_nhwc_f32': (_i, [_p] * 8 + [_i] * 13 + [_p, C.c_size_t, _p]),
    'fgn_winograd_input_f32': (_i, [_p, _p, _p, _p, _i, _i, _i, _i, _i, _i, _p]),
    'fgn_winograd_t_pad': (_i, [_i]),
    'fgn_winograd_gemm_f32': (_i, [_p, _p, _p, _p, _i, _i, _i, _i, _i, _i, _i, _p]),
    'fgn_winograd4_input_f32': (_i, [_p, _p, _p, _p, _i, _i, _i, _i, _i, _i, _p]),
    'fgn_winograd4_output_f32': (_i, [_p, _p, _p, _p, _i, _i, _i, _i, _i, _i, _p]),
    'fgn_winograd_output_f32': (_i, [_p, _p, _p, _p, _i, _i, _i, _i, _i, _i, _p]),
    'fgn_winograd4_variant': (_i, [_i, _i, _i]),
    'fgn_winograd4_index_bits': (_i, [_i] * 11),
    'fgn_winograd4_input_ix_f32': (_i, [_p, _p, _p, _p, _i, _i, _i, _i, _i, _i, _p, _i, _i, _i, _i, _i, _p]),
    'fgn_winograd4_output_ix_f32': (_i, [_p, _p, _p, _p, _i, _i, _i, _i, _i, _i, _p, _i, _i, _i, _i, _i, _p]),
    'fgn_winograd_pack_weights_f32': (_i, [_p, _p, _p, _i, _i, _i, _i, _p]),
    'fgn_winograd4_input2_f32': (_i, [_p, _i, _i, _i, _p, _i, _i, _i, _p, _i, _i, _p]),
    'fgn_winograd4_output2_f32': (_i, [_p, _p, _p, _i, _i, _i, _p, _i, _i, _i, _i, _i, _i, _p]),
    'fgn_nchw3_to_nhwc4_f32': (_i, [_p, _p, _i, _i, _i, _p]),
    'fgn_u8hwc3_to_nhwc4_f32': (_i, [_p, _p, _p, _i, _i, _i, _p]),
    'fgn_resize_u8hwc3_to_nhwc4_f32': (_i, [_p, C.c_longlong, _p, _p, _p, _i, _i, _i, _p]),
    'fgn_resize_mask_u8': (_i, [_p, _p, _i, _i, _i, _i, _i, _p]),
    'fgn_augment_u8hwc3_to_nhwc4_f32': (_i, [_p, C.c_longlong, _p, _p, _p, _i, _i, _i, _p]),
    'fgn_augment_mask_u8': (_i, [_p, _p, _p, _i, _i, _i, _i, _i, _p]),
    'fgn_photometric_u8hwc3': (_i, [_p, _p, C.c_longlong, _p, _i, _p]),
    'fgn_photometric_chain_u8hwc3': (_i, [_p, _p, C.c_longlong, _p, _i, _i, _p]),
    'fgn_support_from_source_f32': (_i, [_p, C.c_longlong, _p, C.c_longlong, _p, _p, _p, _p, _i, _i, _p]),
    'fgn_support_from_source_u8': (_i, [_p, C.c_longlong, _p, C.c_longlong, _p, _p, _p, _i, _i, _p]),
    'fgn_support_augment_f32': (_i, [_p, _p, _p, _p, _p, _p, _i, _i, _p]),
    'fgn_maxpool3x3s2_nhwc_f32': (_i, [_p, _p, _i, _i, _i, _i, _p]),
    'fgn_group_norm_workspace_bytes': (C.c_size_t, [_i] * 4),
    'fgn_group_norm_nhwc_f32': (_i, [_p] * 6 + [C.c_size_t, _i, _i, _i, _i, _f, _i, _p]),
    'fgn_avgpool2x2_nhwc_f32': (_i, [_p, _p, _i, _i, _i, _i, _p]),
    'fgn_roi_align_nhwc_f32': (_i, [_p, _p, _p, _p, _i, _i, _i, _i, _i, _i, _f, _i, _i, _p, _i, _p]),
    'fgn_roi_align2_nhwc_f32': (_i, [_p] * 6 + [_i] * 7 + [_f, _i, _i, _p, _i, _p]),
    'fgn_roi_align_mask_u8': (_i, [_p, _p, _p, _i, _i, _i, _i, _i, _f, _i, _i, _p]),
    'fgn_support_class_vectors_f32': (_i, [_p, _p, _p, _i, _i, _i, _i, _p]),
    'fgn_scale_channels_f32': (_i, [_p, _p, _p, _i, _i, _i, _i, _p]),
    'fgn_support_kmean_f32': (_i, [_p, _p, _i, _i, _i, _i, _p]),
    'fgn_gather_support_vectors_f32': (_i, [_p, _p, _p, _p, _p, _i, _i, _i, _p]),
    'fgn_relation_gn_head_f32': (_i, [_p] * 10 + [_i, _i, _i, _i, _i, _f, _p, _p, _p]),
    'fgn_relation_gn_head_scratch_bytes': (C.c_size_t, [_i, _i, _i]),
    'fgn_gemm_small_f32': (_i, [_p, _p, _p] + [_i] * 7 + [_p]),
    'fgn_rpn_merge_f32': (_i, [_p, _p, _p, _p, _i, _i, _i, _i, _i, _p]),
    'fgn_rpn_proposals_scratch_bytes': (C.c_size_t, [_i, _i, _i]),
    'fgn_rpn_proposals_zeroed_bytes': (C.c_size_t, [_i]),
    'fgn_rpn_proposals_f32': (_i, [_p] * 9 + [_i, _i, _i, _i, _i, _f, _f, C.POINTER(_f), C.POINTER(_f),
                                            _f, _i, _f, _f, _i, _p]),
    'fgn_conv1x1_dual_nhwc_f32': (_i, [_p, _p, _p, _i, _p, _p, _p, _i, _i, _i, _i, _i, _i, _p]),
    'fgn_x3_image_bytes': (C.c_size_t, [_i, _i, _i]),
    'fgn_x3_row_tile': (_i, [C.c_longlong, _i, _i, _i, _i]),
    'fgn_conv1x1_x3_nhwc_f32': (_i, [_p] * 7 + [_i] * 7 + [_p]),
    'fgn_conv1x1_dual_x3_nhwc_f32': (_i, [_p, _p, _p, _i, _p, _p, _p, _i, _i, _i, _i, _i, _i, _p]),
    'fgn_winograd_gemm_x3_f32': (_i, [_p, _p, _p, _p, _i, _i, _i, _i, _i, _i, _i, _p]),
    'fgn_h2_image_bytes': (C.c_size_t, [_i, _i, _i]),
    'fgn_h2_row_tile': (_i, [C.c_longlong, _i, _i, _i, _i]),
    'fgn_h2_k_groups': (_i, [C.c_longlong, _i, _i, _i, _i]),
    'fgn_conv2d_pair_h2_nhwc_f32': (_i, [_p, _i, _i, _i, _p, _i, _i, _i, _p, _p, _p, _p, _p, _i, _i, _i, _i, _i, _i, _i, _i, _p]),
    'fgn_conv2d_pair_h2_bm_nhwc_f32': (_i, [_p, _i, _i, _i, _p, _i, _i, _i, _p, _p, _p, _p, _p, _i, _i, _i, _i, _i, _i, _i, _i, _i, _p]),
    'fgn_gemm_h2_f32': (_i, [_p, _p, _p, _p, _p, _i, _i, _i, _i, _i, _i, _i, _i, _i, _p]),
    'fgn_conv1x1_h2_nhwc_f32': (_i, [_p, _p, _p, _p, _p, _p, _p, _i, _i, _i, _i, _i, _i, _i, _p]),
    'fgn_conv1x1_dual_h2_nhwc_f32': (_i, [_p, _p, _p, _i, _p, _p, _p, _i, _i, _i, _i, _i, _i, _p]),
    'fgn_conv1x1_dual_h2_bm_nhwc_f32': (_i, [_p, _p, _p, _i, _p, _p, _p, _i, _i, _i, _i, _i, _i, _i, _p]),
    'fgn_winograd_gemm_h2_f32': (_i, [_p, _p, _p, _p, _i, _i, _i, _i, _i, _i, _i, _p]),
    'fgn_gemm_x3_f32': (_i, [_p, _p, _p, _p, _p, _i, _i, _i, _i, _i, _i, _i, _i, _i, _i, _p]),
    'fgn_conv2d_pair_nhwc_f32': (_i, [_p, _p, _i, _i, _i, _p, _p, _i, _i, _i, _p, _p, _p] + [_i] * 8 + [_p]),
    'fgn_det_post_scratch_bytes': (C.c_size_t, [_i, _i]),
    'fgn_det_post_f32': (_i, [_p] * 7 + [_i] + [_p] * 3 + [_i, _i, _i, _f, _f, C.POINTER(_f), C.POINTER(_f), _f, _f, _f, _i, _p]),
    'fgn_mask_logits_f32': (_i, [_p, _p, _f, _p, _p, _p, _p, _i, _i, _i, _p]),
    'fgn_mask_paste_u8': (_i, [_p, _p, _i, _p, _p, _i, _i, _i, _i, _f, _i, _p]),
    'fgn_mask_rle': (_i, [_p, _p, _i, _p, _p, _p, _p, _p, _i, _i, _i, _i, _f, _i, _i, _i, _p]),
    'fgn_mask_rle_src': (_i, [_p, _p, _i, _p, _p, _p, _p, _p, _p, _p, _i, _i, _i, _i, _i, _f, _i, _i, _i, _p]),
    'fgn_dense_rle_scratch_bytes': (C.c_size_t, [_i, _i, _i, _i]),
    'fgn_dense_mask_rle': (_i, [_p, _p, C.c_size_t, _p, _p, _p, _i, _i, _i, _i, _i, _p]),
    'fgn_rle_decode_u8': (_i, [_p, C.c_longlong, _p, _p, C.c_longlong, _i, _i, _i, _p]),
    'fgn_color_mask_u8': (_i, [_p, C.c_longlong, C.c_longlong, _i, _p, _i, _p, C.c_longlong, _i, _i, _i, _p]),
    'fgn_poly_masks_u8': (_i, [_p, C.c_longlong, _i, _i, _i, _p, C.c_longlong, _p, C.c_longlong, _i, _i, _p]),
    'fgn_mask_bits_u64': (_i, [_p, _p, _p, _i, _i, _i, _p]),
    'fgn_mask_overlap_i32': (_i, [_p, _p, _i, _p, _p, _p, _p, _i, _i, _i, _i, _i, _f, _i, _p]),
    'fgn_mask_overlap_src_i32': (_i, [_p, _p, _i, _p, _p, _p, _p, _i, _i, _i, _i, _i, _i, _i, _f, _i, _p]),
    'fgn_eval_match_i32': (_i, [_p, _i] + [_p] * 9 + [_i] * 9 + [_p]),
    'fgn_rpn_proposals_large_scratch_bytes': (C.c_size_t, [_i, _i, _i]),
    'fgn_rpn_proposals_large_f32': (_i, [_p] * 7 + [_i, _i, _i, _i, _i, _f, _f, C.POINTER(_f), C.POINTER(_f),
                                                  _f, _i, _f, _f, _i, _p]),
    'fgn_box_assign_scratch_bytes': (C.c_size_t, [_i, _i]),
    'fgn_box_assign_f32': (_i, [_p, _i, _p, _p, _i, _i, _f, _f, _f, _i, _p, _p, _p, _p]),
    'fgn_bbox2delta_f32': (_i, [_p, _p, _p, _i, C.POINTER(_f), C.POINTER(_f), _p]),
    'fgn_bce_logits_sum_f32': (_i, [_p, _p, _p, C.c_longlong, _f, C.c_double, _p, _p]),
    'fgn_smooth_l1_sum_f32': (_i, [_p, _p, _p, C.c_longlong, _f, C.c_double, _p, _p]),
    'fgn_softmax_ce_sum_f32': (_i, [_p, _p, _p, _i, _i, C.c_double, _p, _p]),
    'fgn_bn_train_scratch_bytes': (C.c_size_t, [_i]),
    'fgn_bn_train_f32': (_i, [_p, _i, _i, _p, _p, _f, _f, _p, _p, _p, _i, _p, _p, _p, _p, _p]),
    'fgn_bce_logits_grad_f32': (_i, [_p, _p, _p, C.c_longlong, _f, _f, _p, _p]),
    'fgn_smooth_l1_grad_f32': (_i, [_p, _p, _p, C.c_longlong, _f, _f, _p, _p]),
    'fgn_softmax_ce_grad_f32': (_i, [_p, _p, _p, _i, _i, _f, _p, _p]),
    'fgn_relu_backward_f32': (_i, [_p, _p, _p, C.c_longlong, _p]),
    'fgn_colsum_scratch_bytes': (C.c_size_t, [_i]),
    'fgn_colsum_f32': (_i, [_p, C.c_longlong, _i, _p, _p, _i, _p]),
# ... 53 lines not shown
```

fgn_amd/ops.py:

```python
from __future__ import annotations

import ctypes as C
import math
import os
from dataclasses import dataclass
from typing import Optional

import numpy as np
import torch

from . import lib as _lib


PROFILE = None

FUSED_SHORTCUT = os.environ.get('FGN_FUSED_SHORTCUT', '1') != '0'
GEMM_MATH = os.environ.get('FGN_GEMM_MATH', 'h2')
X3_KERNELS = {64: 'conv_pw_x3_kernel<2, 1, 6, 2, true>', 128: 'conv_pw_x3_kernel<2, 2, 6, 2, true>'}
H2_KERNELS = {64: 'conv_pw_h2_kernel<2, 2, 1, 2, %s, 1>', 128: 'conv_pw_h2_kernel<2, 2, 2, 2, %s, 1>',
              264: 'conv_pw_h2_kernel<4, 1, 1, 2, %s, 1>', 1064: 'conv_pw_h2_kernel<2, 2, 1, 2, %s, 2>'}
H2_BM_KG2 = 1064
H2_DUAL_KERNELS = {64: 'conv_pw_h2_kernel_dual<2, 2, 1, 2, 1>', 128: 'conv_pw_h2_kernel_dual<2, 2, 2, 2, 1>',
                   264: 'conv_pw_h2_kernel_dual<4, 1, 1, 2, 1>', 1064: 'conv_pw_h2_kernel_dual<2, 2, 1, 2, 2>'}

# ... 661 lines not shown
                  relu: bool = False, eps: float = 1e-5, m: Optional[int] = None) -> WinogradLayer:
    m = WINOGRAD_M if m is None else m
    cout, cin, kh, kw = weight.shape
    if (kh, kw) != (3, 3) or cin % 32 != 0 or cout % 4 != 0 or m not in _WG_G:
        raise _lib.FgnHipError('pack_winograd: needs a 3x3 kernel, Cin % 32 == 0, Cout % 4 == 0, m in (2, 4)')
    w = weight.detach().double()
    scale = shift = None
    if bn is not None:
        scale = bn['weight'].double() / torch.sqrt(bn['running_var'].double() + eps)
        shift = bn['bias'].double() - bn['running_mean'].double() * scale
        if bias is not None:
            shift = shift + bias.double() * scale
        w = w * scale[:, None, None, None]
    elif bias is not None:
        shift = bias.detach().double()
    G = _WG_G[m].to(w.device)
    u = torch.einsum('ai,ocij,bj->aboc', G, w, G)
    cout_pad = (cout + 127) // 128 * 128
    up = torch.zeros((m + 2) ** 2, cout_pad, cin, dtype=torch.float32, device=w.device)
    up[:, :cout] = u.reshape((m + 2) ** 2, cout, cin).float()
    return WinogradLayer(up.contiguous(), None if shift is None else shift.float().contiguous(), cin, cout,
                         cout_pad, relu, m, pack_x3(up) if _x3_ok(cin, cout) else None, pack_h2(up) if _h2_ok(cin, cout) else None)


_WG_G_DEV: dict = {}


def repack_conv_(layer: ConvLayer, weight: torch.Tensor, bias: Optional[torch.Tensor] = None) -> ConvLayer:
    cout, cin, kh, kw = weight.shape
    if (cout, cin, kh, kw) != (layer.cout, layer.cin, layer.kh, layer.kw) or cin == 4 or layer.scale is not None:
        raise _lib.FgnHipError('repack_conv_: layer and weight do not match (or the layer folds a BatchNorm)')
    k = kh * kw * cin
    if layer.w.shape[1] == k:
        layer.w[:cout].view(cout, kh, kw, cin).copy_(weight.detach().permute(0, 2, 3, 1))
    else:
        layer.w[:cout, :k].copy_(weight.detach().permute(0, 2, 3, 1).reshape(cout, k))
    if bias is not None:
        layer.shift.copy_(bias.detach())
    if layer.w3 is not None:
        layer.w3.copy_(pack_x3(layer.w))
    if layer.wh is not None:
        layer.wh.copy_(pack_h2(layer.w))
    return layer


def repack_winograd_(layer: WinogradLayer, weight: torch.Tensor, bias: Optional[torch.Tensor] = None) -> WinogradLayer:
    cout, cin, kh, kw = weight.shape
    if (cout, cin, kh, kw) != (layer.cout, layer.cin, 3, 3):
        raise _lib.FgnHipError('repack_winograd_: layer and weight do not match')
    w = weight.detach()
    _chk(w, 'weight')
    key = (layer.m, w.device)
    G = _WG_G_DEV.get(key)
    if G is None:
        G = _WG_G_DEV[key] = _WG_G[layer.m].to(w.device).contiguous()
    rc = _lib.load().fgn_winograd_pack_weights_f32(_ptr(w), _ptr(G), _ptr(layer.u), cout, cin, layer.cout_pad, layer.m,
                                                   _stream())
    _lib.check(rc, 'fgn_winograd_pack_weights_f32')
    if bias is not None:
        layer.shift.copy_(bias.detach())
    if layer.u3 is not None:
        layer.u3.copy_(pack_x3(layer.u))
    if layer.uh is not None:
        layer.uh.copy_(pack_h2(layer.u))
    return layer


def _wg_tiles(H: int, W: int, m: int) -> int:
    return ((H + m - 1) // m) * ((W + m - 1) // m)


def winograd_fits(n_img: int, H: int, W: int, cin: int, cout: int, m: Optional[int] = None) -> bool:
    m = WINOGRAD_M if m is None else m
    t_pad = (n_img * _wg_tiles(H, W, m) + 63) // 64 * 64
    rows = (m + 2) ** 2 * t_pad
    return rows * cin * 4 < 0x7fffff00 and rows * cout < (1 << 31)


def winograd_pays(n_img: int, H: int, W: int, cin: int, cout: int, m: Optional[int] = None) -> bool:
    m = WINOGRAD_M if m is None else m
    return cin >= (_WG_MIN_CIN if m == 4 else 128) and n_img * H * W >= 1024 and winograd_fits(n_img, H, W, cin, cout, m)


def _winograd_gemm(L, layer: WinogradLayer, V, Mo, n_img_dev, n_img: int, tiles: int, t_pad: int, st) -> str:
    route = _gemm_route(L, layer.u3, layer.uh, layer.groups * t_pad, layer.cout, layer.cin, t_pad, n_img * tiles)
    name = 'fgn_winograd_gemm_%sf32' % _ROUTE_INFIX[route]
    u = {'h2': layer.uh, 'x3': layer.u3, 'f32': layer.u}[route]
    _lib.check(getattr(L, name)(_ptr(V), u.data_ptr(), _ptr(Mo), _ptr(n_img_dev), n_img, tiles, t_pad, layer.cin, layer.cout,
                                layer.cout_pad, layer.groups, st), name)
    return route


def _winograd_records(prof, ev, L, layer: WinogradLayer, route: str, t_pad: int, valid: int, tiles: int, pixels: int,
                      bits=(64, 64), **common) -> None:
    G, cin, cout = layer.groups, layer.cin, layer.cout
    kin, kout = 'wg_input_kernel', 'wg_output_kernel'
    if layer.m == 4:
        vi, vo = L.fgn_winograd4_variant(valid, cin, 0), L.fgn_winograd4_variant(valid, cout, 1)
        kin = 'wg4_input_kernel<%d, %s>' % (vi // 10, 'true' if vi % 10 else 'false')
        kout = 'wg4_output_kernel<%d>' % (vo // 10)
        if bits[0] == 32:
            kin = 'wg4_input_narrow_kernel<%d>' % (vi // 10)
        if bits[1] == 32:
            kout = 'wg4_output_narrow_kernel<%d>' % (vo // 10)
    prof.append(dict(kind='wg_in', kernel=kin, e0=ev[0][0], e1=ev[0][1], flop_direct=0.0, flop_issued=0.0, **common))
    gid = L.fgn_conv2d_kernel_id(G * t_pad, 1, 1, cin, cout, layer.cout_pad, 1, 1, 1, 0, 1, 0, 0, 4)
    prof.append(dict(kind='wg_gemm', kernel=_gemm_kernel(route, kernel_name(gid), G * t_pad, cout, cin, t_pad, valid),
                     math=route, e0=ev[1][0], e1=ev[1][1], flop_direct=2.0 * pixels * cout * 9 * cin,
                     flop_issued=2.0 * G * tiles * cout * cin, gemm=(G, tiles, cout, cin), **common))
    prof.append(dict(kind='wg_out', kernel=kout, e0=ev[2][0], e1=ev[2][1], flop_direct=0.0, flop_issued=0.0, **common))


def conv3x3_winograd(x: torch.Tensor, layer: WinogradLayer, in_scale: Optional[torch.Tensor] = None,
                     a_img_div: int = 1, n_img_dev: Optional[torch.Tensor] = None,
                     out: Optional[torch.Tensor] = None) -> torch.Tensor:
    _chk(x, 'x')
    n_in, H, W, cin = x.shape
    if cin != layer.cin:
        raise _lib.FgnHipError(f'conv3x3_winograd: Cin {cin} != layer Cin {layer.cin}')
    n_img = n_in * a_img_div
    if in_scale is not None:
        _chk(in_scale, 'in_scale')
        if tuple(in_scale.shape) != (n_img, cin):
            raise _lib.FgnHipError('conv3x3_winograd: in_scale must be [n_img, Cin]')
    if n_img_dev is not None:
        _chk(n_img_dev, 'n_img_dev', torch.int32)
    tiles = _wg_tiles(H, W, layer.m)
    L = _lib.load()
    f_in, f_out = (L.fgn_winograd4_input_f32, L.fgn_winograd4_output_f32) if layer.m == 4 else \
        (L.fgn_winograd_input_f32, L.fgn_winograd_output_f32)
    G = layer.groups
    t_pad = L.fgn_winograd_t_pad(n_img * tiles)
    V = torch.empty((G, t_pad, cin), device=x.device, dtype=torch.float32)
    Mo = torch.empty((G, t_pad, layer.cout), device=x.device, dtype=torch.float32)
    if out is None:
        y = torch.empty((n_img, H, W, layer.cout), device=x.device, dtype=torch.float32)
    else:
        _chk(out, 'out')
        if tuple(out.shape) != (n_img, H, W, layer.cout):
            raise _lib.FgnHipError('conv3x3_winograd: bad out shape')
        y = out
    prof = PROFILE
    st = _stream()
    ev = [] if prof is not None else None
    if ev is not None:
        ev.append(prof.arm())
    _lib.check(f_in(_ptr(x), _ptr(in_scale), _ptr(V), _ptr(n_img_dev), n_img, a_img_div, H, W, cin, t_pad, st),
               'fgn_winograd_input_f32')
    if ev is not None:
        ev.append(prof.arm())
    route = _winograd_gemm(L, layer, V, Mo, n_img_dev, n_img, tiles, t_pad, st)
    if ev is not None:
        ev.append(prof.arm())
    _lib.check(f_out(_ptr(Mo), _ptr(y), _ptr(layer.shift), _ptr(n_img_dev), n_img, H, W, layer.cout, t_pad,
                     int(layer.relu), st), 'fgn_winograd_output_f32')
    if ev is not None:
        bits = (64, 64) if layer.m != 4 else (
            winograd4_index_bits(n_img, H, W, cin, t_pad, a_img_div=a_img_div, with_scale=in_scale is not None),
            winograd4_index_bits(n_img, H, W, layer.cout, t_pad, output=True))
        _winograd_records(prof, ev, L, layer, route, t_pad, n_img * tiles, tiles, H * W, bits=bits, n_img=n_img, n_img_dev=n_img_dev,
                          shape=(n_img, H, W, cin, layer.cout, 3, 1))
    return y


def winograd4_index_bits(n_img: int, H: int, W: int, C: int, t_pad: int, a_img_div: int = 1, second=None,
                         with_scale: bool = False, output: bool = False) -> int:
    n1, h1, w1 = second if second is not None else (0, 1, 1)
    return _lib.load().fgn_winograd4_index_bits(n_img, a_img_div, H, W, n1, h1, w1, C, t_pad, int(with_scale), int(output))


def winograd4_input(x: torch.Tensor, V: torch.Tensor, in_scale: Optional[torch.Tensor] = None, a_img_div: int = 1,
                    n_img_dev: Optional[torch.Tensor] = None, x1: Optional[torch.Tensor] = None, index_bits: int = 0,
                    vec: int = 0) -> None:
    _chk(x, 'x')
    _chk(V, 'V')
    n_in, H, W, C = x.shape
    n1, h1, w1 = (0, 1, 1) if x1 is None else tuple(x1.shape[:3])
    rc = _lib.load().fgn_winograd4_input_ix_f32(_ptr(x), _ptr(in_scale), _ptr(V), _ptr(n_img_dev), n_in * a_img_div, a_img_div,
                                                H, W, C, V.shape[1], _ptr(x1), n1, h1, w1, index_bits, vec, _stream())
    _lib.check(rc, 'fgn_winograd4_input_ix_f32')


def winograd4_output(Mo: torch.Tensor, y: torch.Tensor, shift: Optional[torch.Tensor] = None, relu: bool = False,
                     n_img_dev: Optional[torch.Tensor] = None, y1: Optional[torch.Tensor] = None, index_bits: int = 0,
                     vec: int = 0) -> None:
    _chk(Mo, 'Mo')
    _chk(y, 'y')
    n, H, W, C = y.shape
    n1, h1, w1 = (0, 1, 1) if y1 is None else tuple(y1.shape[:3])
    rc = _lib.load().fgn_winograd4_output_ix_f32(_ptr(Mo), _ptr(y), _ptr(shift), _ptr(n_img_dev), n, H, W, C, Mo.shape[1],
                                                 int(relu), _ptr(y1), n1, h1, w1, index_bits, vec, _stream())
    _lib.check(rc, 'fgn_winograd4_output_ix_f32')


def conv3x3_winograd_multi(xs, layer: WinogradLayer, outs) -> None:
    L = _lib.load()
    f_in, f_out = (L.fgn_winograd4_input_f32, L.fgn_winograd4_output_f32) if layer.m == 4 else \
        (L.fgn_winograd_input_f32, L.fgn_winograd_output_f32)
    cin, cout, G = layer.cin, layer.cout, layer.groups
    tiles = []
    for x, y in zip(xs, outs):
        _chk(x, 'x')
        _chk(y, 'out')
        if x.shape[-1] != cin or tuple(y.shape) != tuple(x.shape[:-1]) + (cout,):
            raise _lib.FgnHipError('conv3x3_winograd_multi: operand shapes inconsistent')
        tiles.append(x.shape[0] * _wg_tiles(x.shape[1], x.shape[2], layer.m))
    total = sum(tiles)
    t_pad = L.fgn_winograd_t_pad(total)
    if G * t_pad * max(cin, cout) * 4 >= 0x7fffff00:
        raise _lib.FgnHipError('conv3x3_winograd_multi: V / Mo exceed the 2 GiB descriptors')
    dev = xs[0].device
    V = torch.empty((G, t_pad, cin), device=dev, dtype=torch.float32)
    Mo = torch.empty((G, t_pad, cout), device=dev, dtype=torch.float32)
    st = _stream()
    pair = layer.m == 4 and len(xs) == 2
    prof = PROFILE if pair else None
    ev = []
    if prof is not None:
        ev.append(prof.arm())
    if pair:
        (n0, h0, w0, _), (n1, h1, w1, _) = xs[0].shape, xs[1].shape
        _lib.check(L.fgn_winograd4_input2_f32(_ptr(xs[0]), n0, h0, w0, _ptr(xs[1]), n1, h1, w1, _ptr(V), cin, t_pad, st),
                   'fgn_winograd4_input2_f32')
    else:
        off = 0
        for x, n_t in zip(xs, tiles):
            n, H, W, _ = x.shape
            _lib.check(f_in(_ptr(x), None, V.data_ptr() + off * cin * 4, None, n, 1, H, W, cin, t_pad, st),
                       'fgn_winograd_input_f32')
            off += n_t
    if prof is not None:
        ev.append(prof.arm())
    route = _winograd_gemm(L, layer, V, Mo, None, 1, total, t_pad, st)
    if prof is not None:
        ev.append(prof.arm())
    if pair:
        _lib.check(L.fgn_winograd4_output2_f32(_ptr(Mo), _ptr(layer.shift), _ptr(outs[0]), n0, h0, w0, _ptr(outs[1]), n1, h1,
                                               w1, cout, t_pad, int(layer.relu), st), 'fgn_winograd4_output2_f32')
    else:
        off = 0
        for y, n_t in zip(outs, tiles):
            n, H, W, _ = y.shape
            _lib.check(f_out(Mo.data_ptr() + off * cout * 4, _ptr(y), _ptr(layer.shift), None, n, H, W, cout, t_pad,
                             int(layer.relu), st), 'fgn_winograd_output_f32')
            off += n_t
    if prof is not None:
        pixels = sum(x.shape[0] * x.shape[1] * x.shape[2] for x in xs)
        bits = (winograd4_index_bits(n0, h0, w0, cin, t_pad, second=(n1, h1, w1)),
                winograd4_index_bits(n0, h0, w0, cout, t_pad, second=(n1, h1, w1), output=True))
        _winograd_records(prof, ev, L, layer, route, t_pad, total, total, pixels, bits=bits, n_img=1, n_img_dev=None,
                          shape=(len(xs), pixels, 1, cin, cout, 3, 1))


def nchw3_to_nhwc4(x: torch.Tensor) -> torch.Tensor:
    _chk(x, 'x')
    n, c, h, w = x.shape
    if c != 3:
        raise _lib.FgnHipError('nchw3_to_nhwc4: expects 3 channels')
    y = torch.empty((n, h, w, 4), device=x.device, dtype=torch.float32)
    _lib.check(_lib.load().fgn_nchw3_to_nhwc4_f32(_ptr(x), _ptr(y), n, h, w, _stream()),
               'fgn_nchw3_to_nhwc4_f32')
    return y


def input_lut(mean, std, scale: float = 255.0) -> np.ndarray:
    mean, std = np.asarray(mean, np.float32).reshape(3), np.asarray(std, np.float32).reshape(3)
    v = np.arange(256, dtype=np.uint8)[:, None]
    return np.ascontiguousarray(((v.astype(np.float32) / scale - mean) / std).T)


U8_PIXELS_PER_PASS = 256 * 8 * 256 * 4


def u8hwc3_to_nhwc4(x_u8: torch.Tensor, lut: torch.Tensor) -> torch.Tensor:
    _chk(x_u8, 'x_u8', torch.uint8)
# ... 1502 lines not shown
```

include/fgn_hip.h:

```cpp
#ifndef FGN_HIP_H
#define FGN_HIP_H
#include <stddef.h>
#include <stdint.h>

#ifdef __cplusplus
extern "C" {
#endif

#define FGN_OK 0
#define FGN_ERR_SHAPE (-1)
#define FGN_ERR_ARG (-2)

int fgn_abi_version(void);

int fgn_profile_next_launch(void* start_event, void* stop_event);
int fgn_profile_stamp_words(void);
int fgn_profile_stamps(void* records, int capacity);
int fgn_phase_signal(int32_t* counter, void* stream);
int fgn_phase_wait(const int32_t* counter, int32_t target, int timeout_us, void* stream);

size_t fgn_conv2d_workspace_bytes(int n_img, int H, int W, int Cin, int Cout, int KH, int KW, int stride,
                                  int pad, int tile_hint);
int fgn_conv2d_kernel_id(int n_img, int H, int W, int Cin, int Cout, int cout_pad, int KH, int KW, int stride,
                         int pad, int a_img_div, int has_in_scale, int has_residual, int tile_hint);
int fgn_conv2d_nhwc_f32(const float* x, const float* w_packed, float* y, const float* scale,
                        const float* shift, const float* residual, const float* in_scale,
                        const int32_t* n_img_dev, int n_img, int H, int W, int Cin, int Cout,
                        int cout_pad, int KH, int KW, int stride, int pad, int a_img_div, int relu,
                        int tile_hint, float* splitk_ws, size_t splitk_ws_bytes, void* stream);

int fgn_conv1x1_dual_nhwc_f32(const float* x, const float* x2, const int32_t* x2_rows, int x2_total_rows,
                              const float* w_packed, float* y, const float* shift, int rows, int Cin1, int Cin2, int Cout,
                              int cout_pad, int relu, void* stream);

size_t fgn_x3_image_bytes(int K, int npad, int n_groups);
int fgn_x3_row_tile(long long M, int Cout, int K, int grp_rows, int grp_valid);
int fgn_gemm_x3_f32(const float* x, const void* w_x3, float* y, const float* shift, const float* residual, int rows, int K,
                    int Cout, int npad, int relu, int grp_rows, int grp_valid, int n_groups, int bm, int nterms,
                    void* stream);
int fgn_conv1x1_x3_nhwc_f32(const float* x, const void* w_x3, float* y, const float* scale, const float* shift,
                            const float* residual, const int32_t* n_img_dev, int n_img, int H, int W, int Cin, int Cout,
                            int cout_pad, int relu, void* stream);
int fgn_conv1x1_dual_x3_nhwc_f32(const float* x, const float* x2, const int32_t* x2_rows, int x2_total_rows,
                                 const void* w_x3, float* y, const float* shift, int rows, int Cin1, int Cin2, int Cout,
                                 int cout_pad, int relu, void* stream);
int fgn_winograd_gemm_x3_f32(const float* V, const void* U_x3, float* Mo, const int32_t* n_img_dev, int n_img,
                             int tiles_per_img, int t_pad, int Cin, int Cout, int cout_pad, int n_groups, void* stream);
size_t fgn_h2_image_bytes(int K, int npad, int n_groups);
int fgn_h2_k_groups(long long M, int Cout, int K, int grp_rows, int grp_valid);
int fgn_h2_row_tile(long long M, int Cout, int K, int grp_rows, int grp_valid);
int fgn_conv2d_pair_h2_nhwc_f32(const float* x0, int n_img0, int H0, int W0, const float* x1, int n_img1, int H1, int W1,
                                const void* w_h2, float* y0, float* y1, const float* scale, const float* shift, int Cin,
                                int Cout, int cout_pad, int KH, int KW, int stride, int pad, int relu, void* stream);
int fgn_conv2d_pair_h2_bm_nhwc_f32(const float* x0, int n_img0, int H0, int W0, const float* x1, int n_img1, int H1, int W1,
                                   const void* w_h2, float* y0, float* y1, const float* scale, const float* shift, int Cin,
                                   int Cout, int cout_pad, int KH, int KW, int stride, int pad, int relu, int bm, void* stream);
int fgn_gemm_h2_f32(const float* x, const void* w_h2, float* y, const float* shift, const float* residual, int rows, int K,
                    int Cout, int npad, int relu, int grp_rows, int grp_valid, int n_groups, int bm, void* stream);
int fgn_conv1x1_h2_nhwc_f32(const float* x, const void* w_h2, float* y, const float* scale, const float* shift,
                            const float* residual, const int32_t* n_img_dev, int n_img, int H, int W, int Cin, int Cout,
                            int cout_pad, int relu, void* stream);
int fgn_conv1x1_dual_h2_nhwc_f32(const float* x, const float* x2, const int32_t* x2_rows, int x2_total_rows,
                                 const void* w_h2, float* y, const float* shift, int rows, int Cin1, int Cin2, int Cout,
                                 int cout_pad, int relu, void* stream);
int fgn_conv1x1_dual_h2_bm_nhwc_f32(const float* x, const float* x2, const int32_t* x2_rows, int x2_total_rows,
                                    const void* w_h2, float* y, const float* shift, int rows, int Cin1, int Cin2, int Cout,
                                    int cout_pad, int relu, int bm, void* stream);
int fgn_winograd_gemm_h2_f32(const float* V, const void* U_h2, float* Mo, const int32_t* n_img_dev, int n_img,
                             int tiles_per_img, int t_pad, int Cin, int Cout, int cout_pad, int n_groups, void* stream);

int fgn_conv2d_pair_nhwc_f32(const float* x0, float* y0, int n_img0, int H0, int W0, const float* x1, float* y1,
                             int n_img1, int H1, int W1, const float* w_packed, const float* scale, const float* shift,
                             int Cin, int Cout, int cout_pad, int KH, int KW, int stride, int pad, int relu,
                             void* stream);

int fgn_winograd_input_f32(const float* x, const float* in_scale, float* V, const int32_t* n_img_dev, int n_img,
                           int a_img_div, int H, int W, int C, int t_pad, void* stream);
int fgn_winograd_t_pad(int tiles_total);
int fgn_winograd_gemm_f32(const float* V, const float* U, float* Mo, const int32_t* n_img_dev, int n_img,
                          int tiles_per_img, int t_pad, int Cin, int Cout, int cout_pad, int n_groups, void* stream);
int fgn_winograd_output_f32(const float* Mo, float* y, const float* shift, const int32_t* n_img_dev, int n_img,
                            int H, int W, int C, int t_pad, int relu, void* stream);
int fgn_winograd4_input_f32(const float* x, const float* in_scale, float* V, const int32_t* n_img_dev, int n_img,
                            int a_img_div, int H, int W, int C, int t_pad, void* stream);
int fgn_winograd4_output_f32(const float* Mo, float* y, const float* shift, const int32_t* n_img_dev, int n_img,
                             int H, int W, int C, int t_pad, int relu, void* stream);
int fgn_winograd4_input2_f32(const float* x0, int n_img0, int H0, int W0, const float* x1, int n_img1, int H1, int W1,
                             float* V, int C, int t_pad, void* stream);
int fgn_winograd4_output2_f32(const float* Mo, const float* shift, float* y0, int n_img0, int H0, int W0, float* y1,
                              int n_img1, int H1, int W1, int C, int t_pad, int relu, void* stream);
int fgn_winograd4_index_bits(int n_img, int a_img_div, int H, int W, int n_img1, int H1, int W1, int C, int t_pad,
                             int with_scale, int is_output);
int fgn_winograd4_input_ix_f32(const float* x, const float* in_scale, float* V, const int32_t* n_img_dev, int n_img,
                               int a_img_div, int H, int W, int C, int t_pad, const float* x1, int n_img1, int H1, int W1,
                               int index_bits, int vec, void* stream);
int fgn_winograd4_output_ix_f32(const float* Mo, float* y, const float* shift, const int32_t* n_img_dev, int n_img, int H,
                                int W, int C, int t_pad, int relu, float* y1, int n_img1, int H1, int W1, int index_bits,
                                int vec, void* stream);
int fgn_winograd4_variant(int tiles_total, int C, int is_output);
int fgn_winograd_pack_weights_f32(const float* w, const double* G, float* U, int cout, int cin, int cout_pad, int m,
                                  void* stream);

int fgn_nchw3_to_nhwc4_f32(const float* x, float* y, int n_img, int H, int W, void* stream);

int fgn_u8hwc3_to_nhwc4_f32(const unsigned char* x, const float* lut, float* y, int n_img, int H, int W, void* stream);

int fgn_resize_u8hwc3_to_nhwc4_f32(const unsigned char* src, long long src_stride_bytes, const int* src_hw,
                                   const float* lut, float* y, int n_img, int H, int W, void* stream);
int fgn_resize_mask_u8(const unsigned char* src, unsigned char* dst, int G, int h, int w, int H, int W, void* stream);

int fgn_augment_u8hwc3_to_nhwc4_f32(const unsigned char* src, long long src_stride_bytes, const int* recs,
                                    const float* lut, float* y, int n_img, int H, int W, void* stream);
int fgn_augment_mask_u8(const unsigned char* src, unsigned char* dst, const int* rec, int G, int h, int w, int H, int W,
                        void* stream);

int fgn_photometric_u8hwc3(const unsigned char* src, unsigned char* dst, long long stride_bytes, const int* recs,
                           int n_img, void* stream);

int fgn_photometric_chain_u8hwc3(const unsigned char* src, unsigned char* dst, long long stride_bytes, const int* recs,
                                 int n_ops, int n_img, void* stream);

int fgn_support_from_source_f32(const unsigned char* src, long long src_stride_bytes, const unsigned char* msk,
                                long long msk_stride_bytes, const int* recs, const float* lut, float* y,
                                unsigned char* m, int n, int S, void* stream);

int fgn_support_from_source_u8(const unsigned char* src, long long src_stride_bytes, const unsigned char* msk,
                               long long msk_stride_bytes, const int* recs, unsigned char* crop, unsigned char* m,
                               int n, int S, void* stream);

int fgn_support_augment_f32(const unsigned char* crop, const unsigned char* msk, const int* recs, const float* lut,
                            float* y, unsigned char* m, int n, int S, void* stream);

int fgn_maxpool3x3s2_nhwc_f32(const float* x, float* y, int n_img, int H, int W, int C, void* stream);

size_t fgn_group_norm_workspace_bytes(int n_img, int HW, int C, int groups);
int fgn_group_norm_nhwc_f32(const float* x, float* y, const float* gamma, const float* beta,
                            const float* residual, void* ws, size_t ws_bytes, int n_img, int HW, int C,
                            int groups, float eps, int relu, void* stream);

int fgn_avgpool2x2_nhwc_f32(const float* x, float* y, int n_img, int H, int W, int C, void* stream);

int fgn_roi_align_nhwc_f32(const float* fmap, const float* rois, float* out, const int32_t* n_rois_dev,
                           int n_rois, int n_img, int H, int W, int C, int out_size, float spatial_scale,
                           int sampling_ratio, int aligned, const float* post_shift, int relu, void* stream);
int fgn_roi_align2_nhwc_f32(const float* fmap, const float* fmap2, const float* rois, float* out, float* out2,
                            const int32_t* n_rois_dev, int n_rois, int n_img, int H, int W, int C, int C2,
                            int out_size, float spatial_scale, int sampling_ratio, int aligned,
                            const float* post_shift2, int relu2, void* stream);
int fgn_roi_align_mask_u8(const uint8_t* mask, const float* rois, float* out, int n_rois, int n_img, int H,
                          int W, int out_size, float spatial_scale, int sampling_ratio, int aligned,
                          void* stream);

int fgn_support_class_vectors_f32(const float* x, const float* weights, float* out, int n_groups, int K,
                                  int P, int C, void* stream);
int fgn_support_kmean_f32(const float* x, float* out, int n_groups, int K, int P, int C, void* stream);
int fgn_gather_support_vectors_f32(const float* table, const int64_t* labels, const float* rois, float* out,
                                   const int32_t* n_dev, int n, int n_ways, int C, void* stream);

int fgn_scale_channels_f32(const float* x, const float* v, float* out, int n_out, int div, int P, int C,
                           void* stream);

int fgn_relation_gn_head_f32(const float* Q, const float* S, const float* rois, const float* gn_weight,
                             const float* gn_bias, const float* fc_weight, const float* fc_bias, float* cls_out,
                             float* reg_out, const int32_t* n_rois_dev, int n_rois, int n_ways, int C,
                             int gn_groups, int roi_size, float eps, float* rel_out_debug, float* scratch, void* stream);
size_t fgn_relation_gn_head_scratch_bytes(int n_rois, int n_ways, int C);

int fgn_rpn_merge_f32(const float* head, float* logits, float* scores, float* deltas, int batch, int n_ways,
                      int HW, int n_anchors, int head_channels, void* stream);

size_t fgn_rpn_proposals_scratch_bytes(int batch, int n_total, int nms_pre);
size_t fgn_rpn_proposals_zeroed_bytes(int batch);
int fgn_rpn_proposals_f32(const float* scores, const float* deltas, const float* base_anchors, void* scratch,
                          void* pre_zeroed, float* proposals, float* rois_out, int32_t* n_props, int32_t* dbg_topk_idx, int batch, int feat_h,
                          int feat_w, int n_anchors, int stride, float img_h, float img_w,
                          const float* host_means4, const float* host_stds4, float max_ratio, int nms_pre,
                          float min_bbox_size, float iou_thr, int max_per_img, void* stream);

size_t fgn_det_post_scratch_bytes(int max_rois, int n_ways);
int fgn_det_post_f32(const float* rois, const float* cls_raw, const float* reg_raw, const int32_t* n_rois_dev,
                     void* scratch, float* det_bboxes, float* mask_rois_out , int img_index, int64_t* det_labels, int32_t* n_dets,
// ... 145 lines not shown
```

Baseline: 341.6 img/s.

## Compact Winograd F(4,3) transform groups to skip provably-zero edge tile products

Adds a compact layout for F(4x4,3x3) Winograd. In the 36 transform groups, the last row/column components of partial edge tiles are not stored, so each group has its own row count. The input/output transform kernels and the pointwise GEMM kernels use a packed per-group tile-count descriptor, which lets GEMM tiles skip rows that do not exist. The Python conv3x3_winograd path turns this on by default for m=4 layers. This cuts GEMM work and transform memory traffic for images whose size is not a multiple of 4, at the cost of more index arithmetic and branching in the transforms and tile-activity checks.

```diff
diff --git a/fgn_amd/csrc/common.h b/fgn_amd/csrc/common.h
--- a/fgn_amd/csrc/common.h
+++ b/fgn_amd/csrc/common.h
@@ -46,6 +46,18 @@
     return e;
 }
 
+struct Wg4Compact {
+    int ty, tx, ty_f, tx_f;
+    __host__ __device__ int rows(int a, int b) const { return (a == 5 ? ty_f : ty) * (b == 5 ? tx_f : tx); }
+};
+static inline Wg4Compact wg4_compact(int H, int W) {
+    Wg4Compact c;
+    c.ty = (H + 3) / 4; c.tx = (W + 3) / 4;
+    c.ty_f = (H % 4 == 0) ? c.ty : c.ty - 1;
+    c.tx_f = (W % 4 == 0) ? c.tx : c.tx - 1;
+    return c;
+}
+
 typedef float f32x16 __attribute__((ext_vector_type(16)));
 typedef float f32x4 __attribute__((ext_vector_type(4)));
 
diff --git a/fgn_amd/csrc/conv_igemm.hip b/fgn_amd/csrc/conv_igemm.hip
--- a/fgn_amd/csrc/conv_igemm.hip
+++ b/fgn_amd/csrc/conv_igemm.hip
@@ -26,6 +26,7 @@
     unsigned x_bytes = 0, w_bytes = 0;
     int grp_rows = 0, grp_valid = 0, grp_items = 0, grp_rows_per_item = 0, grp_w_stride = 0;
     const int32_t* grp_count_dev = nullptr;
+    unsigned grp_compact = 0u;
     unsigned long long* stamp = nullptr;
     const float* x2 = nullptr;
     unsigned x2_bytes = 0;
@@ -36,6 +37,27 @@
     int npad3 = 0;
     const float* w_inv = nullptr;
 };
+
+struct ConvGrpCounts {
+    int full, items;
+};
+__device__ __forceinline__ ConvGrpCounts conv_grp_counts(const ConvParams& p) {
+    ConvGrpCounts c;
+    c.full = p.grp_valid;
+    c.items = p.grp_items;
+    if (p.grp_rows && p.grp_count_dev) {
+        c.items = min(p.grp_items, *p.grp_count_dev);
+        c.full = min(c.full, c.items * p.grp_rows_per_item);
+    }
+    return c;
+}
+__device__ __forceinline__ int conv_grp_valid(const ConvParams& p, int grp, const ConvGrpCounts& c) {
+    if (!p.grp_compact) return c.full;
+    const int a = grp / 6, b = grp - a * 6;
+    const int tx = (int)(p.grp_compact & 0x7fffu), ty = (int)((p.grp_compact >> 15) & 0x7fffu);
+    const int nx = (b == 5) ? tx - (int)((p.grp_compact >> 30) & 1u) : tx, ny = (a == 5) ? ty - (int)(p.grp_compact >> 31) : ty;
+    return c.items * ny * nx;
+}
 
 #ifndef CONV_DMA_STAGES
 #define CONV_DMA_STAGES 2
@@ -453,8 +475,7 @@
     int b_off0 = ((n0 + row0) * p.K + src_c4 * 4) * 4;
     if (PW && p.grp_rows) {
         const int grp = m0 / p.grp_rows;
-        int valid = p.grp_valid;
-        if (p.grp_count_dev) valid = min(valid, min(p.grp_items, *p.grp_count_dev) * p.grp_rows_per_item);
+        const int valid = conv_grp_valid(p, grp, conv_grp_counts(p));
         if (m0 - grp * p.grp_rows >= valid) return;
         b_off0 += grp * p.grp_w_stride * 4;
     }
@@ -708,8 +729,7 @@
     const int t = threadIdx.x, lane = t & 63, wv = t >> 6;
     const int wm = wv >> 1, wn = wv & 1;
     const int M = (p.n_img_dev ? min(p.n_img, *p.n_img_dev) : p.n_img) * p.Ho * p.Wo;
-    int grp_valid = p.grp_valid;
-    if (p.grp_rows && p.grp_count_dev) grp_valid = min(grp_valid, min(p.grp_items, *p.grp_count_dev) * p.grp_rows_per_item);
+    const ConvGrpCounts grp_counts = conv_grp_counts(p);
 
     const int col4 = t & 7, row0 = t >> 3;
     const int src_c4 = col4 ^ ((row0 >> 1) & 7);
@@ -742,7 +762,10 @@
         m0 = tile_m * BM;
         n0 = tile_n * BN;
         if (m0 >= M) return false;
-        if (p.grp_rows && m0 - (m0 / p.grp_rows) * p.grp_rows >= grp_valid) return false;
+        if (p.grp_rows) {
+            const int grp = m0 / p.grp_rows;
+            if (m0 - grp * p.grp_rows >= conv_grp_valid(p, grp, grp_counts)) return false;
+        }
         return true;
     };
     auto next_active = [&](int tile, int& m0, int& n0) -> int {
@@ -1553,9 +1576,15 @@
 
 static int describe_winograd_gemm(ConvParams& p, const GemmMath& m, const float* V, const void* U, float* Mo,
                                   const int32_t* n_img_dev, int n_img, int tiles_per_img, int t_pad, int Cin, int Cout,
-                                  int cout_pad, int n_groups) {
+                                  int cout_pad, int n_groups, int H = 0, int W = 0) {
     if (!V || !U || !Mo) return FGN_ERR_ARG;
     if (n_img <= 0) return FGN_OK;
+    if (H < 0 || W < 0 || (H > 0) != (W > 0)) return FGN_ERR_SHAPE;
+    if (H > 0) {
+        const Wg4Compact c = wg4_compact(H, W);
+        if (n_groups != 36 || tiles_per_img != c.ty * c.tx || c.ty > 0x7fff || c.tx > 0x7fff) return FGN_ERR_SHAPE;
+        p.grp_compact = (unsigned)c.tx | (unsigned)c.ty << 15 | (unsigned)(c.tx_f < c.tx) << 30 | (unsigned)(c.ty_f < c.ty) << 31;
+    }
     if (Cin % BK != 0 || (m.deep && Cin < 2 * BK) || Cout % 4 != 0 || cout_pad % m.bn != 0 || cout_pad < Cout || t_pad % 64 != 0 ||
         (n_groups != 16 && n_groups != 36) || (long long)n_img * tiles_per_img > t_pad)
         return FGN_ERR_SHAPE;
@@ -1603,3 +1632,29 @@
     if (rc != FGN_DESCRIBED) return rc;
     return launch_h2(p, p.n_img, n_groups, 0, stream);
 }
+
+static int wg4c_tiles(int H, int W) { return H > 0 && W > 0 ? ((H + 3) / 4) * ((W + 3) / 4) : 0; }
+extern "C" int fgn_winograd4c_gemm_f32(const float* V, const float* U, float* Mo, const int32_t* n_img_dev, int n_img, int H,
+                                       int W, int t_pad, int Cin, int Cout, int cout_pad, hipStream_t stream) {
+    ConvParams p;
+    if (H < 1 || W < 1) return FGN_ERR_SHAPE;
+    const int rc = describe_winograd_gemm(p, MATH_F32, V, U, Mo, n_img_dev, n_img, wg4c_tiles(H, W), t_pad, Cin, Cout, cout_pad, 36, H, W);
+    if (rc != FGN_DESCRIBED) return rc;
+    return launch_cfg<64, 64, 32, 32, 4>(p, p.n_img, pointwise_mode(4, p.n_img, Cout, 1), stream);
+}
+extern "C" int fgn_winograd4c_gemm_x3_f32(const float* V, const void* U_x3, float* Mo, const int32_t* n_img_dev, int n_img,
+                                          int H, int W, int t_pad, int Cin, int Cout, int cout_pad, hipStream_t stream) {
+    ConvParams p;
+    if (H < 1 || W < 1) return FGN_ERR_SHAPE;
+    const int rc = describe_winograd_gemm(p, MATH_X3, V, U_x3, Mo, n_img_dev, n_img, wg4c_tiles(H, W), t_pad, Cin, Cout, cout_pad, 36, H, W);
+    if (rc != FGN_DESCRIBED) return rc;
+    return launch_x3(p, p.n_img, 0, 6, stream);
+}
+extern "C" int fgn_winograd4c_gemm_h2_f32(const float* V, const void* U_h2, float* Mo, const int32_t* n_img_dev, int n_img,
+                                          int H, int W, int t_pad, int Cin, int Cout, int cout_pad, hipStream_t stream) {
+    ConvParams p;
+    if (H < 1 || W < 1) return FGN_ERR_SHAPE;
+    const int rc = describe_winograd_gemm(p, MATH_H2, V, U_h2, Mo, n_img_dev, n_img, wg4c_tiles(H, W), t_pad, Cin, Cout, cout_pad, 36, H, W);
+    if (rc != FGN_DESCRIBED) return rc;
+    return launch_h2(p, p.n_img, 36, 0, stream);
+}
diff --git a/fgn_amd/csrc/conv_pw_h2.h b/fgn_amd/csrc/conv_pw_h2.h
--- a/fgn_amd/csrc/conv_pw_h2.h
+++ b/fgn_amd/csrc/conv_pw_h2.h
@@ -119,8 +119,8 @@
     const int tg = KG == 1 ? t : t % NTHR_G;
     const int wm = wv / WNW, wn = wv % WNW;
     const int M = IM2COL ? q2.M0 + q2.M1 : (p.n_img_dev ? min(p.n_img, *p.n_img_dev) : p.n_img) * p.Ho * p.Wo;
-    int grp_valid = p.grp_valid;
-    if (p.grp_rows && p.grp_count_dev) grp_valid = min(grp_valid, min(p.grp_items, *p.grp_count_dev) * p.grp_rows_per_item);
+    ConvGrpCounts grp_counts = {0, 0};
+    if constexpr (!IM2COL) grp_counts = conv_grp_counts(p);
 
     float a_s = 1.f, a_inv = 1.f;
 
@@ -156,7 +156,12 @@
         m0 = tile_m * BM;
         n0 = tile_n * BN;
         if (m0 >= M) return false;
-        if (p.grp_rows && m0 - (m0 / p.grp_rows) * p.grp_rows >= grp_valid) return false;
+        if constexpr (!IM2COL) {
+            if (p.grp_rows) {
+                const int grp = m0 / p.grp_rows;
+                if (m0 - grp * p.grp_rows >= conv_grp_valid(p, grp, grp_counts)) return false;
+            }
+        }
         return true;
     };
     auto next_active = [&](int tile, int& m0, int& n0) -> int {
@@ -176,7 +181,11 @@
     auto offsets = [&](int m0, int n0) -> Offs {
         Offs o;
         o.a2[0] = 0u;
-        const int g_end = p.grp_rows ? (m0 / p.grp_rows) * p.grp_rows + grp_valid : M;
+        int g_end = M;
+        if (p.grp_rows) {
+            const int grp = m0 / p.grp_rows;
+            g_end = grp * p.grp_rows + conv_grp_valid(p, grp, grp_counts);
+        }
 #pragma unroll
         for (int i = 0; i < A_LD; ++i) {
             const int m = m0 + row0 + ROWS_PER_PASS * i;
diff --git a/fgn_amd/csrc/conv_pw_x3.h b/fgn_amd/csrc/conv_pw_x3.h
--- a/fgn_amd/csrc/conv_pw_x3.h
+++ b/fgn_amd/csrc/conv_pw_x3.h
@@ -53,8 +53,7 @@
     const int t = threadIdx.x, lane = t & 63, wv = t >> 6;
     const int wm = wv >> 1, wn = wv & 1;
     const int M = (p.n_img_dev ? min(p.n_img, *p.n_img_dev) : p.n_img) * p.Ho * p.Wo;
-    int grp_valid = p.grp_valid;
-    if (p.grp_rows && p.grp_count_dev) grp_valid = min(grp_valid, min(p.grp_items, *p.grp_count_dev) * p.grp_rows_per_item);
+    const ConvGrpCounts grp_counts = conv_grp_counts(p);
 
     const int col4 = t & 7, row0 = t >> 3;
     const int src_c4 = col4 ^ ((row0 >> 1) & 7);
@@ -88,7 +87,10 @@
         m0 = tile_m * BM;
         n0 = tile_n * BN;
         if (m0 >= M) return false;
-        if (p.grp_rows && m0 - (m0 / p.grp_rows) * p.grp_rows >= grp_valid) return false;
+        if (p.grp_rows) {
+            const int grp = m0 / p.grp_rows;
+            if (m0 - grp * p.grp_rows >= conv_grp_valid(p, grp, grp_counts)) return false;
+        }
         return true;
     };
     auto next_active = [&](int tile, int& m0, int& n0) -> int {
diff --git a/fgn_amd/csrc/winograd.hip b/fgn_amd/csrc/winograd.hip
--- a/fgn_amd/csrc/winograd.hip
+++ b/fgn_amd/csrc/winograd.hip
@@ -191,7 +191,22 @@
     int tiles0;
 };
 
-template <int V, bool EAGER>
+struct Wg4cRows {
+    size_t r[2][2];
+    bool row_ok, col_ok;
+};
+__device__ __forceinline__ Wg4cRows wg4c_rows(int img, int yy, int xx, int ty, int tx, int ty_f, int tx_f) {
+    Wg4cRows q;
+    q.r[0][0] = ((size_t)img * ty + yy) * tx + xx;
+    q.r[0][1] = ((size_t)img * ty + yy) * tx_f + xx;
+    q.r[1][0] = ((size_t)img * ty_f + yy) * tx + xx;
+    q.r[1][1] = ((size_t)img * ty_f + yy) * tx_f + xx;
+    q.row_ok = yy < ty_f;
+    q.col_ok = xx < tx_f;
+    return q;
+}
+
+template <int V, bool EAGER, bool COMPACT = false>
 __global__ __launch_bounds__(256) void wg4_input_kernel(const float* __restrict__ x_, const float* __restrict__ in_scale_,
                                                         float* __restrict__ V_, const int32_t* __restrict__ n_img_dev,
                                                         int n_img, int a_img_div, int H, int W, int CV, int ty, int tx,
@@ -264,8 +279,20 @@
                 for (int a = 0; a < 6; ++a) tt[a][b] = rr[a];
             }
         }
+        const size_t gs = (size_t)t_pad * CV;
+        if constexpr (COMPACT) {
+            const Wg4cRows q = wg4c_rows(img, yy, xx, ty, tx, seg.ty, seg.tx);
+#pragma unroll
+            for (int a = 0; a < 6; ++a) {
+                T rr[6];
+                wg4_bt<V>(tt[a], rr);
+#pragma unroll
+                for (int b = 0; b < 6; ++b)
+                    if ((a < 5 || q.row_ok) && (b < 5 || q.col_ok)) Vo[(a * 6 + b) * gs + q.r[a == 5][b == 5] * CV + c] = rr[b];
+            }
+            continue;
+        }
         T* dst = Vo + (size_t)t * CV + c;
-        const size_t gs = (size_t)t_pad * CV;
 #pragma unroll
         for (int a = 0; a < 6; ++a) {
             T rr[6];
@@ -276,7 +303,7 @@
     }
 }
 
-template <int V>
+template <int V, bool COMPACT = false>
 __global__ __launch_bounds__(256) void wg4_output_kernel(const float* __restrict__ Mo_, float* __restrict__ y_,
                                                          const float* __restrict__ shift_,
                                                          const int32_t* __restrict__ n_img_dev, int n_img, int H, int W,
@@ -308,10 +335,20 @@
         const T* src = Mo + (size_t)t * CV + c;
         const size_t gs = (size_t)t_pad * CV;
         T mm[6][6];
-#pragma unroll
-        for (int a = 0; a < 6; ++a)
-#pragma unroll
-            for (int b = 0; b < 6; ++b) mm[a][b] = src[(a * 6 + b) * gs];
+        if constexpr (COMPACT) {
+            const Wg4cRows q = wg4c_rows(img, yy, xx, ty, tx, seg.ty, seg.tx);
+#pragma unroll
+            for (int a = 0; a < 6; ++a)
+#pragma unroll
+                for (int b = 0; b < 6; ++b)
+                    mm[a][b] = ((a < 5 || q.row_ok) && (b < 5 || q.col_ok))
+                                   ? Mo[(a * 6 + b) * gs + q.r[a == 5][b == 5] * CV + c] : vzero<V>();
+        } else {
+#pragma unroll
+            for (int a = 0; a < 6; ++a)
+#pragma unroll
+                for (int b = 0; b < 6; ++b) mm[a][b] = src[(a * 6 + b) * gs];
+        }
         T st[4][6];
 #pragma unroll
         for (int b = 0; b < 6; ++b) {
@@ -370,7 +407,23 @@
     uint32_t CV;
     WgDiv dcv, ddiv;
     uint32_t gs;
+    uint32_t ty_f, tx_f;
 };
+struct Wg4cOffs {
+    uint32_t o[2][2];
+    bool row_ok, col_ok;
+};
+__device__ __forceinline__ Wg4cOffs wg4c_offs(uint32_t img, uint32_t yy, uint32_t xx, uint32_t ty, uint32_t tx, uint32_t ty_f,
+                                              uint32_t tx_f, uint32_t CV, uint32_t c, uint32_t vbytes) {
+    Wg4cOffs q;
+    q.o[0][0] = (((img * ty + yy) * tx + xx) * CV + c) * vbytes;
+    q.o[0][1] = (((img * ty + yy) * tx_f + xx) * CV + c) * vbytes;
+    q.o[1][0] = (((img * ty_f + yy) * tx + xx) * CV + c) * vbytes;
+    q.o[1][1] = (((img * ty_f + yy) * tx_f + xx) * CV + c) * vbytes;
+    q.row_ok = yy < ty_f;
+    q.col_ok = xx < tx_f;
+    return q;
+}
 
 template <typename T>
 __device__ __forceinline__ T wg_ld(const void* base, uint32_t off) {
@@ -388,7 +441,7 @@
     return *p;
 }
 
-template <int V>
+template <int V, bool COMPACT = false>
 __global__ __launch_bounds__(256) void wg4_input_narrow_kernel(const WgNarrow P, const float* __restrict__ in_scale,
                                                                float* __restrict__ Vo, const int32_t* __restrict__ n_img_dev) {
     typedef vf<V> T;
@@ -440,6 +493,21 @@
         for (int a = 0; a < 6; ++a) tt[a][b] = rr[a];
     }
     if ((int)img >= min(n_cap, dev_count)) return;
+    if constexpr (COMPACT) {
+        const Wg4cOffs q = wg4c_offs(img, yy, xx, ty, tx, P.ty_f, P.tx_f, P.CV, c, (uint32_t)sizeof(T));
+        uint32_t go = 0u;
+#pragma unroll
+        for (int a = 0; a < 6; ++a) {
+            T rr[6];
+            wg4_bt<V>(tt[a], rr);
+#pragma unroll
+            for (int b = 0; b < 6; ++b) {
+                if ((a < 5 || q.row_ok) && (b < 5 || q.col_ok)) wg_st<T>(Vo, q.o[a == 5][b == 5] + go, rr[b]);
+                go += P.gs;
+            }
+        }
+        return;
+    }
     uint32_t o = (t * P.CV + c) * (uint32_t)sizeof(T);
 #pragma unroll
     for (int a = 0; a < 6; ++a) {
@@ -453,7 +521,7 @@
     }
 }
 
-template <int V>
+template <int V, bool COMPACT = false>
 __global__ __launch_bounds__(256) void wg4_output_narrow_kernel(const WgNarrow P, const float* __restrict__ Mo,
                                                                 const float* __restrict__ shift,
                                                                 const int32_t* __restrict__ n_img_dev, int relu) {
@@ -471,7 +539,20 @@
     const uint32_t tl = wg_quot(i, P.dcv), c = i - tl * P.CV;
     const uint32_t t = tl + (second ? P.tiles0 : 0u);
     T mm[6][6];
-    {
+    if constexpr (COMPACT) {
+        const uint32_t r_ = wg_quot(tl, dtx), xx_ = tl - r_ * tx;
+        const uint32_t img_ = wg_quot(r_, dty), yy_ = r_ - img_ * ty;
+        const Wg4cOffs q = wg4c_offs(img_, yy_, xx_, ty, tx, P.ty_f, P.tx_f, P.CV, c, (uint32_t)sizeof(T));
+#pragma unroll
+        for (int a = 0; a < 5; ++a)
+#pragma unroll
+            for (int b = 0; b < 5; ++b) mm[a][b] = wg_ld<T>(Mo, q.o[0][0] + (uint32_t)(a * 6 + b) * P.gs);
+#pragma unroll
+        for (int a = 0; a < 5; ++a) mm[a][5] = q.col_ok ? wg_ld<T>(Mo, q.o[0][1] + (uint32_t)(a * 6 + 5) * P.gs) : vzero<V>();
+#pragma unroll
+        for (int b = 0; b < 5; ++b) mm[5][b] = q.row_ok ? wg_ld<T>(Mo, q.o[1][0] + (uint32_t)(30 + b) * P.gs) : vzero<V>();
+        mm[5][5] = (q.row_ok && q.col_ok) ? wg_ld<T>(Mo, q.o[1][1] + 35u * P.gs) : vzero<V>();
+    } else {
         uint32_t o = (t * P.CV + c) * (uint32_t)sizeof(T);
 #pragma unroll
         for (int a = 0; a < 6; ++a)
@@ -545,7 +626,9 @@
     P.dcv = wg_div(P.CV);
     P.ddiv = wg_div((uint32_t)a_img_div);
     P.gs = (uint32_t)t_pad * (uint32_t)C * 4u;
-    *grid = (int)(P.blocks0 + (P.m[1].elems + 255u) / 256u);
+    const Wg4Compact cl = wg4_compact(H0, W0);
+    P.ty_f = (uint32_t)cl.ty_f; P.tx_f = (uint32_t)cl.tx_f;
+    *grid =(int)(P.blocks0 + (P.m[1].elems + 255u) / 256u);
     return P;
 }
 static bool wg4_takes_narrow(bool is_output, int n_img, int a_img_div, int H, int W, int n_img1, int H1, int W1, int C,
@@ -567,11 +650,17 @@
                      a_img_div, H, W, C / VV, ty, tx, t_pad, total, seg)
 #define WG4_IN_NARROW(VV)                                                                                              \
     FGN_LAUNCH_TIMED((wg4_input_narrow_kernel<VV>), dim3(ngrid), dim3(256), 0, stream, P, in_scale, V, n_img_dev)
+#define WG4C_IN_LAUNCH(VV)                                                                                             \
+    FGN_LAUNCH_TIMED((wg4_input_kernel<VV, true, true>), dim3(grid), dim3(256), 0, stream, x, in_scale, V, n_img_dev, \
+                     n_img, a_img_div, H, W, C / VV, ty, tx, t_pad, total, seg)
+#define WG4C_IN_NARROW(VV)                                                                                             \
+    FGN_LAUNCH_TIMED((wg4_input_narrow_kernel<VV, true>), dim3(ngrid), dim3(256), 0, stream, P, in_scale, V, n_img_dev)
 
 static int wg4_input_launch(const float* x, const float* in_scale, float* V, const int32_t* n_img_dev, int n_img,
                             int a_img_div, int H, int W, int C, int t_pad, const float* x1, int n_img1, int H1, int W1,
-                            int index_bits, int vec_force, hipStream_t stream) {
+                            int index_bits, int vec_force, hipStream_t stream, bool compact = false) {
     if (!x || !V) return FGN_ERR_ARG;
+    if (compact && x1) return FGN_ERR_ARG;
     if (index_bits != 0 && index_bits != 32 && index_bits != 64) return FGN_ERR_ARG;
     if (vec_force != 0 && vec_force != 1 && vec_force != 2 && vec_force != 4) return FGN_ERR_ARG;
     if (n_img <= 0) return FGN_OK;
@@ -590,15 +679,29 @@
     if (fits && index_bits != 64) {
         int ngrid = 0;
         const WgNarrow P = wg4_narrow(x, n_img, a_img_div, H, W, x1, n_img1, H1, W1, C, vec, t_pad, &ngrid);
-        switch (vec) {
+        switch (vec + (compact ? 10 : 0)) {
             case 1: WG4_IN_NARROW(1); break;
             case 2: WG4_IN_NARROW(2); break;
-            default: WG4_IN_NARROW(4); break;
+            case 4: WG4_IN_NARROW(4); break;
+            case 11: WG4C_IN_NARROW(1); break;
+            case 12: WG4C_IN_NARROW(2); break;
+            default: WG4C_IN_NARROW(4); break;
         }
         FGN_LAUNCH_CHECK();
         return FGN_OK;
     }
     const int grid = (int)std::min<long long>((total + 255) / 256, 256 * 32);
+    if (compact) {
+        const Wg4Compact cl = wg4_compact(H, W);
+        seg.ty = cl.ty_f; seg.tx = cl.tx_f;
+        switch (vec) {
+            case 1: WG4C_IN_LAUNCH(1); break;
+            case 2: WG4C_IN_LAUNCH(2); break;
+            default: WG4C_IN_LAUNCH(4); break;
+        }
+        FGN_LAUNCH_CHECK();
+        return FGN_OK;
+    }
     switch (vec * 10 + (eager ? 1 : 0)) {
         case 11: WG4_IN_LAUNCH(1, true); break;
         case 10: WG4_IN_LAUNCH(1, false); break;
@@ -627,16 +730,36 @@
                             x1 ? W1 : 1, index_bits, vec, stream);
 }
 
-#define WG4_OUT_LAUNCH(VV)                                                                                             \
+extern "C" int fgn_winograd4c_input_f32(const float* x, const float* in_scale, float* V, const int32_t* n_img_dev, int n_img,
+                                        int a_img_div, int H, int W, int C, int t_pad, int index_bits, int vec,
+                                        hipStream_t stream) {
+    return wg4_input_launch(x, in_scale, V, n_img_dev, n_img, a_img_div, H, W, C, t_pad, nullptr, 0, 1, 1, index_bits, vec, stream, true);
+}
+extern "C" int fgn_winograd4c_group_rows(int n_img, int H, int W, int* rows36) {
+    if (!rows36) return FGN_ERR_ARG;
+    if (n_img < 0 || H < 1 || W < 1) return FGN_ERR_SHAPE;
+    const Wg4Compact cl = wg4_compact(H, W);
+    for (int a = 0; a < 6; ++a)
+        for (int b = 0; b < 6; ++b) rows36[a * 6 + b] = n_img * cl.rows(a, b);
+    return FGN_OK;
+}
+
+#define WG4_OUT_LAUNCH(VV)                                                                                            \
     FGN_LAUNCH_TIMED((wg4_output_kernel<VV>), dim3(grid), dim3(256), 0, stream, Mo, y, shift, n_img_dev, n_img, H, W, \
                      C / VV, ty, tx, t_pad, relu, total, seg)
 #define WG4_OUT_NARROW(VV)                                                                                             \
     FGN_LAUNCH_TIMED((wg4_output_narrow_kernel<VV>), dim3(ngrid), dim3(256), 0, stream, P, Mo, shift, n_img_dev, relu)
+#define WG4C_OUT_LAUNCH(VV)                                                                                            \
+    FGN_LAUNCH_TIMED((wg4_output_kernel<VV, true>), dim3(grid), dim3(256), 0, stream, Mo, y, shift, n_img_dev, n_img, H, \
+                     W, C / VV, ty, tx, t_pad, relu, total, seg)
+#define WG4C_OUT_NARROW(VV)                                                                                            \
+    FGN_LAUNCH_TIMED((wg4_output_narrow_kernel<VV, true>), dim3(ngrid), dim3(256), 0, stream, P, Mo, shift, n_img_dev, relu)
 
 static int wg4_output_launch(const float* Mo, float* y, const float* shift, const int32_t* n_img_dev, int n_img, int H,
                              int W, int C, int t_pad, int relu, float* y1, int n_img1, int H1, int W1, int index_bits,
-                             int vec_force, hipStream_t stream) {
+                             int vec_force, hipStream_t stream, bool compact = false) {
     if (!Mo || !y) return FGN_ERR_ARG;
+    if (compact && y1) return FGN_ERR_ARG;
     if (index_bits != 0 && index_bits != 32 && index_bits != 64) return FGN_ERR_ARG;
     if (vec_force != 0 && vec_force != 1 && vec_force != 2 && vec_force != 4) return FGN_ERR_ARG;
     if (n_img <= 0) return FGN_OK;
@@ -654,15 +777,29 @@
     if (fits && index_bits != 64) {
         int ngrid = 0;
         const WgNarrow P = wg4_narrow(y, n_img, 1, H, W, y1, n_img1, H1, W1, C, vec, t_pad, &ngrid);
-        switch (vec) {
+        switch (vec + (compact ? 10 : 0)) {
             case 1: WG4_OUT_NARROW(1); break;
             case 2: WG4_OUT_NARROW(2); break;
-            default: WG4_OUT_NARROW(4); break;
+            case 4: WG4_OUT_NARROW(4); break;
+            case 11: WG4C_OUT_NARROW(1); break;
+            case 12: WG4C_OUT_NARROW(2); break;
+            default: WG4C_OUT_NARROW(4); break;
         }
         FGN_LAUNCH_CHECK();
         return FGN_OK;
     }
     const int grid = (int)std::min<long long>((total + 255) / 256, 256 * 32);
+    if (compact) {
+        const Wg4Compact cl = wg4_compact(H, W);
+        seg.ty = cl.ty_f; seg.tx = cl.tx_f;
+        switch (vec) {
+            case 1: WG4C_OUT_LAUNCH(1); break;
+            case 2: WG4C_OUT_LAUNCH(2); break;
+            default: WG4C_OUT_LAUNCH(4); break;
+        }
+        FGN_LAUNCH_CHECK();
+        return FGN_OK;
+    }
     switch (vec) {
         case 1: WG4_OUT_LAUNCH(1); break;
         case 2: WG4_OUT_LAUNCH(2); break;
@@ -687,6 +824,11 @@
                                            int H1, int W1, int index_bits, int vec, hipStream_t stream) {
     return wg4_output_launch(Mo, y, shift, n_img_dev, n_img, H, W, C, t_pad, relu, y1, y1 ? n_img1 : 0, y1 ? H1 : 1,
                              y1 ? W1 : 1, index_bits, vec, stream);
+}
+extern "C" int fgn_winograd4c_output_f32(const float* Mo, float* y, const float* shift, const int32_t* n_img_dev, int n_img,
+                                         int H, int W, int C, int t_pad, int relu, int index_bits, int vec,
+                                         hipStream_t stream) {
+    return wg4_output_launch(Mo, y, shift, n_img_dev, n_img, H, W, C, t_pad, relu, nullptr, 0, 1, 1, index_bits, vec, stream, true);
 }
 
 template <int R>
diff --git a/fgn_amd/lib.py b/fgn_amd/lib.py
--- a/fgn_amd/lib.py
+++ b/fgn_amd/lib.py
@@ -30,6 +30,12 @@
     'fgn_winograd4_index_bits': (_i, [_i] * 11),
     'fgn_winograd4_input_ix_f32': (_i, [_p, _p, _p, _p, _i, _i, _i, _i, _i, _i, _p, _i, _i, _i, _i, _i, _p]),
     'fgn_winograd4_output_ix_f32': (_i, [_p, _p, _p, _p, _i, _i, _i, _i, _i, _i, _p, _i, _i, _i, _i, _i, _p]),
+    'fgn_winograd4c_group_rows': (_i, [_i, _i, _i, _p]),
+    'fgn_winograd4c_input_f32': (_i, [_p, _p, _p, _p, _i, _i, _i, _i, _i, _i, _i, _i, _p]),
+    'fgn_winograd4c_output_f32': (_i, [_p, _p, _p, _p, _i, _i, _i, _i, _i, _i, _i, _i, _p]),
+    'fgn_winograd4c_gemm_f32': (_i, [_p, _p, _p, _p, _i, _i, _i, _i, _i, _i, _i, _p]),
+    'fgn_winograd4c_gemm_x3_f32': (_i, [_p, _p, _p, _p, _i, _i, _i, _i, _i, _i, _i, _p]),
+    'fgn_winograd4c_gemm_h2_f32': (_i, [_p, _p, _p, _p, _i, _i, _i, _i, _i, _i, _i, _p]),
     'fgn_winograd_pack_weights_f32': (_i, [_p, _p, _p, _i, _i, _i, _i, _p]),
     'fgn_winograd4_input2_f32': (_i, [_p, _i, _i, _i, _p, _i, _i, _i, _p, _i, _i, _p]),
     'fgn_winograd4_output2_f32': (_i, [_p, _p, _p, _i, _i, _i, _p, _i, _i, _i, _i, _i, _i, _p]),
diff --git a/fgn_amd/ops.py b/fgn_amd/ops.py
--- a/fgn_amd/ops.py
+++ b/fgn_amd/ops.py
@@ -767,17 +767,28 @@
     return cin >= (_WG_MIN_CIN if m == 4 else 128) and n_img * H * W >= 1024 and winograd_fits(n_img, H, W, cin, cout, m)
 
 
-def _winograd_gemm(L, layer: WinogradLayer, V, Mo, n_img_dev, n_img: int, tiles: int, t_pad: int, st) -> str:
+def winograd4_group_rows(n_img: int, H: int, W: int) -> list:
+    rows = (C.c_int * 36)()
+    _lib.check(_lib.load().fgn_winograd4c_group_rows(n_img, H, W, rows), 'fgn_winograd4c_group_rows')
+    return list(rows)
+
+
+def _winograd_gemm(L, layer: WinogradLayer, V, Mo, n_img_dev, n_img: int, tiles: int, t_pad: int, st, compact_hw=None) -> str:
     route = _gemm_route(L, layer.u3, layer.uh, layer.groups * t_pad, layer.cout, layer.cin, t_pad, n_img * tiles)
+    u = {'h2': layer.uh, 'x3': layer.u3, 'f32': layer.u}[route]
+    if compact_hw is not None:
+        name = 'fgn_winograd4c_gemm_%sf32' % _ROUTE_INFIX[route]
+        _lib.check(getattr(L, name)(_ptr(V), u.data_ptr(), _ptr(Mo), _ptr(n_img_dev), n_img, compact_hw[0], compact_hw[1], t_pad,
+                                    layer.cin, layer.cout, layer.cout_pad, st), name)
+        return route
     name = 'fgn_winograd_gemm_%sf32' % _ROUTE_INFIX[route]
-    u = {'h2': layer.uh, 'x3': layer.u3, 'f32': layer.u}[route]
     _lib.check(getattr(L, name)(_ptr(V), u.data_ptr(), _ptr(Mo), _ptr(n_img_dev), n_img, tiles, t_pad, layer.cin, layer.cout,
                                 layer.cout_pad, layer.groups, st), name)
     return route
 
 
 def _winograd_records(prof, ev, L, layer: WinogradLayer, route: str, t_pad: int, valid: int, tiles: int, pixels: int,
-                      bits=(64, 64), **common) -> None:
+                      bits=(64, 64), products: Optional[int] = None, **common) -> None:
     G, cin, cout = layer.groups, layer.cin, layer.cout
     kin, kout = 'wg_input_kernel', 'wg_output_kernel'
     if layer.m == 4:
@@ -788,17 +799,20 @@
             kin = 'wg4_input_narrow_kernel<%d>' % (vi // 10)
         if bits[1] == 32:
             kout = 'wg4_output_narrow_kernel<%d>' % (vo // 10)
+        if products is not None:
+            kin, kout = kin[:-1] + ', true>', kout[:-1] + ', true>'
     prof.append(dict(kind='wg_in', kernel=kin, e0=ev[0][0], e1=ev[0][1], flop_direct=0.0, flop_issued=0.0, **common))
     gid = L.fgn_conv2d_kernel_id(G * t_pad, 1, 1, cin, cout, layer.cout_pad, 1, 1, 1, 0, 1, 0, 0, 4)
     prof.append(dict(kind='wg_gemm', kernel=_gemm_kernel(route, kernel_name(gid), G * t_pad, cout, cin, t_pad, valid),
                      math=route, e0=ev[1][0], e1=ev[1][1], flop_direct=2.0 * pixels * cout * 9 * cin,
-                     flop_issued=2.0 * G * tiles * cout * cin, gemm=(G, tiles, cout, cin), **common))
+                     flop_issued=2.0 * (G * tiles if products is None else products) * cout * cin, gemm=(G, tiles, cout, cin),
+                     **common))
     prof.append(dict(kind='wg_out', kernel=kout, e0=ev[2][0], e1=ev[2][1], flop_direct=0.0, flop_issued=0.0, **common))
 
 
 def conv3x3_winograd(x: torch.Tensor, layer: WinogradLayer, in_scale: Optional[torch.Tensor] = None,
                      a_img_div: int = 1, n_img_dev: Optional[torch.Tensor] = None,
-                     out: Optional[torch.Tensor] = None) -> torch.Tensor:
+                     out: Optional[torch.Tensor] = None, compact: bool = True) -> torch.Tensor:
     _chk(x, 'x')
     n_in, H, W, cin = x.shape
     if cin != layer.cin:
@@ -830,20 +844,30 @@
     ev = [] if prof is not None else None
     if ev is not None:
         ev.append(prof.arm())
-    _lib.check(f_in(_ptr(x), _ptr(in_scale), _ptr(V), _ptr(n_img_dev), n_img, a_img_div, H, W, cin, t_pad, st),
-               'fgn_winograd_input_f32')
+    compact = compact and layer.m == 4
+    if compact:
+        _lib.check(L.fgn_winograd4c_input_f32(_ptr(x), _ptr(in_scale), _ptr(V), _ptr(n_img_dev), n_img, a_img_div, H, W, cin,
+                                              t_pad, 0, 0, st), 'fgn_winograd4c_input_f32')
+    else:
+        _lib.check(f_in(_ptr(x), _ptr(in_scale), _ptr(V), _ptr(n_img_dev), n_img, a_img_div, H, W, cin, t_pad, st),
+                   'fgn_winograd_input_f32')
     if ev is not None:
         ev.append(prof.arm())
-    route = _winograd_gemm(L, layer, V, Mo, n_img_dev, n_img, tiles, t_pad, st)
+    route = _winograd_gemm(L, layer, V, Mo, n_img_dev, n_img, tiles, t_pad, st, compact_hw=(H, W) if compact else None)
     if ev is not None:
         ev.append(prof.arm())
-    _lib.check(f_out(_ptr(Mo), _ptr(y), _ptr(layer.shift), _ptr(n_img_dev), n_img, H, W, layer.cout, t_pad,
-                     int(layer.relu), st), 'fgn_winograd_output_f32')
+    if compact:
+        _lib.check(L.fgn_winograd4c_output_f32(_ptr(Mo), _ptr(y), _ptr(layer.shift), _ptr(n_img_dev), n_img, H, W, layer.cout,
+                                               t_pad, int(layer.relu), 0, 0, st), 'fgn_winograd4c_output_f32')
+    else:
+        _lib.check(f_out(_ptr(Mo), _ptr(y), _ptr(layer.shift), _ptr(n_img_dev), n_img, H, W, layer.cout, t_pad,
+                         int(layer.relu), st), 'fgn_winograd_output_f32')
     if ev is not None:
         bits = (64, 64) if layer.m != 4 else (
             winograd4_index_bits(n_img, H, W, cin, t_pad, a_img_div=a_img_div, with_scale=in_scale is not None),
             winograd4_index_bits(n_img, H, W, layer.cout, t_pad, output=True))
-        _winograd_records(prof, ev, L, layer, route, t_pad, n_img * tiles, tiles, H * W, bits=bits, n_img=n_img, n_img_dev=n_img_dev,
+        _winograd_records(prof, ev, L, layer, route, t_pad, n_img * tiles, tiles, H * W, bits=bits,
+                          products=sum(winograd4_group_rows(1, H, W)) if compact else None, n_img=n_img, n_img_dev=n_img_dev,
                           shape=(n_img, H, W, cin, layer.cout, 3, 1))
     return y
 
@@ -876,6 +900,26 @@
     rc = _lib.load().fgn_winograd4_output_ix_f32(_ptr(Mo), _ptr(y), _ptr(shift), _ptr(n_img_dev), n, H, W, C, Mo.shape[1],
                                                  int(relu), _ptr(y1), n1, h1, w1, index_bits, vec, _stream())
     _lib.check(rc, 'fgn_winograd4_output_ix_f32')
+
+
+def winograd4c_input(x: torch.Tensor, V: torch.Tensor, in_scale: Optional[torch.Tensor] = None, a_img_div: int = 1,
+                     n_img_dev: Optional[torch.Tensor] = None, index_bits: int = 0, vec: int = 0) -> None:
+    _chk(x, 'x')
+    _chk(V, 'V')
+    n_in, H, W, C_ = x.shape
+    rc = _lib.load().fgn_winograd4c_input_f32(_ptr(x), _ptr(in_scale), _ptr(V), _ptr(n_img_dev), n_in * a_img_div, a_img_div,
+                                              H, W, C_, V.shape[1], index_bits, vec, _stream())
+    _lib.check(rc, 'fgn_winograd4c_input_f32')
+
+
+def winograd4c_output(Mo: torch.Tensor, y: torch.Tensor, shift: Optional[torch.Tensor] = None, relu: bool = False,
+                      n_img_dev: Optional[torch.Tensor] = None, index_bits: int = 0, vec: int = 0) -> None:
+    _chk(Mo, 'Mo')
+    _chk(y, 'y')
+    n, H, W, C_ = y.shape
+    rc = _lib.load().fgn_winograd4c_output_f32(_ptr(Mo), _ptr(y), _ptr(shift), _ptr(n_img_dev), n, H, W, C_, Mo.shape[1],
+                                               int(relu), index_bits, vec, _stream())
+    _lib.check(rc, 'fgn_winograd4c_output_f32')
 
 
 def conv3x3_winograd_multi(xs, layer: WinogradLayer, outs) -> None:
diff --git a/include/fgn_hip.h b/include/fgn_hip.h
--- a/include/fgn_hip.h
+++ b/include/fgn_hip.h
@@ -97,6 +97,17 @@
 int fgn_winograd4_output_ix_f32(const float* Mo, float* y, const float* shift, const int32_t* n_img_dev, int n_img, int H,
                                 int W, int C, int t_pad, int relu, float* y1, int n_img1, int H1, int W1, int index_bits,
                                 int vec, void* stream);
+int fgn_winograd4c_group_rows(int n_img, int H, int W, int* rows36);
+int fgn_winograd4c_input_f32(const float* x, const float* in_scale, float* V, const int32_t* n_img_dev, int n_img,
+                             int a_img_div, int H, int W, int C, int t_pad, int index_bits, int vec, void* stream);
+int fgn_winograd4c_output_f32(const float* Mo, float* y, const float* shift, const int32_t* n_img_dev, int n_img, int H,
+                              int W, int C, int t_pad, int relu, int index_bits, int vec, void* stream);
+int fgn_winograd4c_gemm_f32(const float* V, const float* U, float* Mo, const int32_t* n_img_dev, int n_img, int H, int W,
+                            int t_pad, int Cin, int Cout, int cout_pad, void* stream);
+int fgn_winograd4c_gemm_x3_f32(const float* V, const void* U_x3, float* Mo, const int32_t* n_img_dev, int n_img, int H,
+                               int W, int t_pad, int Cin, int Cout, int cout_pad, void* stream);
+int fgn_winograd4c_gemm_h2_f32(const float* V, const void* U_h2, float* Mo, const int32_t* n_img_dev, int n_img, int H,
+                               int W, int t_pad, int Cin, int Cout, int cout_pad, void* stream);
 int fgn_winograd4_variant(int tiles_total, int C, int is_output);
 int fgn_winograd_pack_weights_f32(const float* w, const double* G, float* U, int cout, int cin, int cout_pad, int m,
                                   void* stream);
```

Result: no change. 344.9 img/s, median of 6 (+1.0%).
